# sony/aki

Measured on NVIDIA B200. Metric: mma_attn_fwd_bwd_tflops, higher is better.
Workload: dtype bf16

## Files before the change

### aki_b200/csrc/attn_bwd_sm100.cu

```cuda
#include <math.h>
#include <stdio.h>
#include <stdlib.h>
#include <mutex>
#include "attn_aux.cuh"
#include "sm100_ptx.cuh"

namespace aki {

namespace bwd {
constexpr int BN = 128, BM = 128;
constexpr int ATOM_BYTES = 128 * 64;
constexpr int TILE_BYTES = 3 * ATOM_BYTES;
constexpr int AUG_BYTES = 128 * 16;
constexpr int DQ_ATOM_BYTES = 128 * 128;
constexpr int Q_STAGES = 2, DO_STAGES = 2;
constexpr int THREADS = 512;
constexpr int MAX_TILES = 512;
constexpr int SMEM_K = 0;
constexpr int SMEM_V = SMEM_K + TILE_BYTES;
constexpr int SMEM_Q = SMEM_V + TILE_BYTES;
constexpr int SMEM_DO = SMEM_Q + Q_STAGES * TILE_BYTES;
constexpr int SMEM_DS = SMEM_DO + DO_STAGES * TILE_BYTES;
constexpr int SMEM_DQ = SMEM_DS + 4 * ATOM_BYTES;
constexpr int SMEM_QAUG = SMEM_DQ + 2 * DQ_ATOM_BYTES;
constexpr int SMEM_ONES = SMEM_QAUG + Q_STAGES * AUG_BYTES;
constexpr int SMEM_ONES_D = SMEM_ONES + 128;
constexpr int SMEM_ZERO = SMEM_ONES_D + 128;
constexpr int SLOTS = 2;
constexpr int SMEM_QLIST = SMEM_ZERO + 128;
constexpr int SMEM_TOTAL = SMEM_QLIST + SLOTS * MAX_TILES * 2;
#ifndef AKI_BWD_SLICES_PER_GROUP
#define AKI_BWD_SLICES_PER_GROUP 8
#endif
constexpr int SMEM_ALLOC = SMEM_TOTAL + 1024;
static_assert(SMEM_ALLOC + 256 <= 232448, "shared memory budget");
constexpr uint32_t TM_S = 0, TM_DP = 128, TM_DV = 256, TM_DK = 352, TM_P = 448;
constexpr int REGS_CTRL = 64, REGS_COMPUTE = 168, REGS_DRAIN = 112;
}

struct BwdKernelParams {
  TensorView d_k, d_v;
  const float* rope_cos;
  const float* rope_sin;
  int64_t rope_stride_b;
  MaskMeta mm;
  int B, H, T, n_t, n_words;
  int group, n_items, use_clc;
  float scale_log2, scale;
  unsigned long long* trace;
  int trace_cta;
};

#ifdef AKI_FWD_TRACE
#define TRB(slot, j, k) do { if (tracing && (j) < 64) P.trace[((slot) * 64 + (j)) * 8 + (k)] = clock64(); } while (0)
#else
#define TRB(slot, j, k) do { } while (0)
#endif

__device__ __forceinline__ void f32x2_mul(float& lo, float& hi, float a_lo, float a_hi, float b_lo, float b_hi) {
  uint64_t r;
  asm("mul.rn.f32x2 %0, %1, %2;" : "=l"(r) : "l"(f32x2_pack(a_lo, a_hi)), "l"(f32x2_pack(b_lo, b_hi)));
  asm("mov.b64 {%0, %1}, %2;" : "=f"(lo), "=f"(hi) : "l"(r));
}

__global__ void __launch_bounds__(bwd::THREADS, 1)
attn_bwd_sm100_kernel(const __grid_constant__ CUtensorMap map_q, const __grid_constant__ CUtensorMap map_k,
                      const __grid_constant__ CUtensorMap map_v, const __grid_constant__ CUtensorMap map_do,
                      const __grid_constant__ CUtensorMap map_dq, const __grid_constant__ CUtensorMap map_qaug,
                      const BwdKernelParams P) {
  using namespace bwd;
  extern __shared__ uint8_t smem_raw[];
  const uint32_t smem_base = (smem_u32(smem_raw) + 1023u) & ~1023u;
  uint8_t* const smem_gen = smem_raw + (smem_base - smem_u32(smem_raw));
  constexpr int KV_FULL = 0, KV_EMPTY = 1, Q_FULL = 2, Q_EMPTY = Q_FULL + Q_STAGES, DO_FULL = Q_EMPTY + Q_STAGES,
                DO_EMPTY = DO_FULL + DO_STAGES, S_FULL = DO_EMPTY + DO_STAGES, P_READY = S_FULL + 1,
                DP_FULL = P_READY + 1, DS_READY = DP_FULL + 1, DQ_FULL = DS_READY + 1, DQ_DRAINED = DQ_FULL + 1,
                ALL_DONE = DQ_DRAINED + 1, ACC_FREE = ALL_DONE + 1,
                ITEM_FULL = ACC_FREE + 1, ITEM_EMPTY = ITEM_FULL + SLOTS, CLC_BAR = ITEM_EMPTY + SLOTS, N_BARS = CLC_BAR + 1;
  __shared__ __align__(8) uint64_t bars[N_BARS];
  __shared__ __align__(16) int4 item_ring[SLOTS][2];
  __shared__ __align__(16) uint4 clc_resp;
  __shared__ uint32_t tmem_base_s;
  const uint32_t bar0 = smem_u32(bars);
  auto BAR = [&](int i) { return bar0 + 8u * i; };

  const int tid = threadIdx.x, warp = tid >> 5, lane = tid & 31;
  uint16_t* const qlist_all = reinterpret_cast<uint16_t*>(smem_gen + SMEM_QLIST);

  if (tid == 0) {
    mbar_init(BAR(KV_FULL), 1); mbar_init(BAR(KV_EMPTY), 2);
    for (int i = 0; i < Q_STAGES; ++i) { mbar_init(BAR(Q_FULL + i), 1); mbar_init(BAR(Q_EMPTY + i), 2); }
    for (int i = 0; i < DO_STAGES; ++i) { mbar_init(BAR(DO_FULL + i), 1); mbar_init(BAR(DO_EMPTY + i), 2); }
    mbar_init(BAR(S_FULL), 1); mbar_init(BAR(P_READY), 256); mbar_init(BAR(DP_FULL), 1);
    mbar_init(BAR(DS_READY), 256); mbar_init(BAR(DQ_FULL), 1); mbar_init(BAR(DQ_DRAINED), 128);
    mbar_init(BAR(ALL_DONE), 2); mbar_init(BAR(ACC_FREE), 256);
    for (int i = 0; i < SLOTS; ++i) { mbar_init(BAR(ITEM_FULL + i), 1); mbar_init(BAR(ITEM_EMPTY + i), 15); }
    mbar_init(BAR(CLC_BAR), 1);
    fence_barrier_init();
  }
  if (warp == 2) {
    tmem_alloc<512>(smem_u32(&tmem_base_s));
    if (lane < 8) *reinterpret_cast<uint4*>(smem_gen + SMEM_ONES + lane * 16) = make_uint4(0x3f803f80u, 0x00003f80u, 0u, 0u);
    else if (lane < 16) *reinterpret_cast<uint4*>(smem_gen + SMEM_ONES_D + (lane - 8) * 16) = make_uint4(0u, 0u, 0x3f803f80u, 0x00003f80u);
    else if (lane < 24) *reinterpret_cast<uint4*>(smem_gen + SMEM_ZERO + (lane - 16) * 16) = make_uint4(0u, 0u, 0u, 0u);
    fence_proxy_async_smem();
  }
  if (warp == 0 && elect_one()) {
    tma_prefetch_desc(&map_q); tma_prefetch_desc(&map_k); tma_prefetch_desc(&map_v); tma_prefetch_desc(&map_do);
    tma_prefetch_desc(&map_dq); tma_prefetch_desc(&map_qaug);
  }
  tc_fence_before();
  __syncthreads();
  tc_fence_after();
  const uint32_t tmem = tmem_base_s;

  auto item_wait = [&](uint32_t n, int4& v0, int4& v1) {
    const int slot = n % SLOTS;
    mbar_wait(BAR(ITEM_FULL + slot), (n / SLOTS) & 1);
    v0 = item_ring[slot][0]; v1 = item_ring[slot][1];
  };

  if (warp == 0) {
    setmaxnreg_dec<REGS_CTRL>();
    if (elect_one()) {
      uint32_t n_it = 0, n_work = 0, qc = 0;
      for (;;) {
        int4 v0, v1;
        item_wait(n_it, v0, v1);
        if (!v0.x) break;
        const int b = v0.y, h = v0.z, j0 = v0.w * BN, n_q = v1.x;
        const uint16_t* qlist = qlist_all + (n_it % SLOTS) * MAX_TILES;
        auto load_tile = [&](int it) {
          const int i0 = (int)qlist[it];
          const uint32_t c = qc + it, sq = c % Q_STAGES, sd = c % DO_STAGES;
          mbar_wait(BAR(Q_EMPTY + sq), ((c / Q_STAGES) & 1) ^ 1);
#ifdef KO_TMA
          if (c >= Q_STAGES) { mbar_arrive(BAR(Q_FULL + sq)); mbar_wait(BAR(DO_EMPTY + sd), ((c / DO_STAGES) & 1) ^ 1); mbar_arrive(BAR(DO_FULL + sd)); return; }
#endif
          mbar_arrive_expect_tx(BAR(Q_FULL + sq), TILE_BYTES + AUG_BYTES);
          for (int a = 0; a < 3; ++a)
            tma_load_4d(smem_base + SMEM_Q + sq * TILE_BYTES + a * ATOM_BYTES, &map_q, BAR(Q_FULL + sq), a * 32, i0, h, b);
          tma_load_4d(smem_base + SMEM_QAUG + sq * AUG_BYTES, &map_qaug, BAR(Q_FULL + sq), 0, i0, h, b);
          mbar_wait(BAR(DO_EMPTY + sd), ((c / DO_STAGES) & 1) ^ 1);
          mbar_arrive_expect_tx(BAR(DO_FULL + sd), TILE_BYTES);
          for (int a = 0; a < 3; ++a)
            tma_load_4d(smem_base + SMEM_DO + sd * TILE_BYTES + a * ATOM_BYTES, &map_do, BAR(DO_FULL + sd), a * 32, i0, h, b);
        };
        if (n_q > 0) {
          const int pre = min(n_q, Q_STAGES);
          for (int it = 0; it < pre; ++it) load_tile(it);
          if (n_work > 0) mbar_wait(BAR(KV_EMPTY), (n_work - 1) & 1);
          mbar_arrive_expect_tx(BAR(KV_FULL), 2 * TILE_BYTES);
          for (int a = 0; a < 3; ++a) {
            tma_load_4d(smem_base + SMEM_K + a * ATOM_BYTES, &map_k, BAR(KV_FULL), a * 32, j0, h, b);
            tma_load_4d(smem_base + SMEM_V + a * ATOM_BYTES, &map_v, BAR(KV_FULL), a * 32, j0, h, b);
          }
          for (int it = pre; it < n_q; ++it) load_tile(it);
          qc += n_q;
          ++n_work;
        }
        mbar_arrive(BAR(ITEM_EMPTY + n_it % SLOTS));
        ++n_it;
      }
    }
  } else if (warp == 1 || warp == 2) {
    setmaxnreg_dec<REGS_CTRL>();
    if (elect_one()) {
      constexpr uint32_t IDESC_SS_KK = umma_idesc_bf16(128, 128, 0, 0);
      constexpr uint32_t IDESC_N96_BMN = umma_idesc_bf16(128, 96, 0, 1);
      constexpr uint32_t IDESC_N96_AMN_BMN = umma_idesc_bf16(128, 96, 1, 1);
      const uint32_t sK = smem_base + SMEM_K, sV = smem_base + SMEM_V, sDS = smem_base + SMEM_DS;
      const uint64_t DESC_KMAJ = umma_smem_desc(0, 16, 512, UMMA_SW64);
      const uint64_t DESC_MNMAJ = umma_smem_desc(0, ATOM_BYTES, 512, UMMA_SW64);
      const uint64_t DESC_ONES = umma_smem_desc(smem_base + SMEM_ONES, SMEM_ZERO - SMEM_ONES, 0, UMMA_SW_NONE);
      const uint64_t DESC_ONES_D = umma_smem_desc(smem_base + SMEM_ONES_D, SMEM_ZERO - SMEM_ONES_D, 0, UMMA_SW_NONE);
      const uint64_t DESC_AUG = umma_smem_desc(0, 0, 128, UMMA_SW_NONE);
      auto kmajor = [&](uint32_t base, int k) {
        return DESC_KMAJ | (uint64_t)(((base + (k >> 1) * ATOM_BYTES + (k & 1) * 32) >> 4) & 0x3FFFu);
      };
      auto mnmajor = [&](uint32_t base, int k) {
        return DESC_MNMAJ | (uint64_t)(((base + k * 1024) >> 4) & 0x3FFFu);
      };
      uint32_t n_it = 0, n_work = 0, gs = 0;
      if (warp == 1) {
        for (;;) {
          int4 v0, v1;
          item_wait(n_it, v0, v1);
          if (!v0.x) break;
          const int n_q = v1.x;
#ifdef AKI_FWD_TRACE
          const bool tracing = P.trace && (int)blockIdx.x == P.trace_cta && n_it == 0;
#endif
          if (n_q > 0) {
          auto issue_s = [&](int it) {
            const uint32_t c = gs + it;
            const uint32_t sQ = smem_base + SMEM_Q + (c % Q_STAGES) * TILE_BYTES;
            const uint32_t sA = smem_base + SMEM_QAUG + (c % Q_STAGES) * AUG_BYTES;
#ifndef KO_S
#pragma unroll
            for (int k = 0; k < 6; ++k) umma_ss(tmem + TM_S, kmajor(sK, k), kmajor(sQ, k), IDESC_SS_KK, k > 0);
            umma_ss(tmem + TM_S, DESC_ONES, DESC_AUG | (uint64_t)((sA >> 4) & 0x3FFFu), IDESC_SS_KK, 1);
#endif
            umma_commit(BAR(S_FULL));
            umma_commit(BAR(Q_EMPTY + c % Q_STAGES));
          };
          mbar_wait(BAR(KV_FULL), n_work & 1);
          mbar_wait(BAR(Q_FULL + gs % Q_STAGES), (gs / Q_STAGES) & 1);
          tc_fence_after();
          issue_s(0);
          for (int it = 0; it < n_q; ++it) {
            const uint32_t c = gs + it;
            const uint32_t sDO = smem_base + SMEM_DO + (c % DO_STAGES) * TILE_BYTES;
            TRB(2, it, 0);
            mbar_wait(BAR(DO_FULL + c % DO_STAGES), (c / DO_STAGES) & 1);
            mbar_wait(BAR(P_READY), c & 1);
            if (it == 0 && n_work > 0) mbar_wait(BAR(ACC_FREE), (n_work - 1) & 1);
            tc_fence_after();
            TRB(2, it, 1);
#ifndef KO_DV
#pragma unroll
            for (int k = 0; k < 8; ++k)
              umma_ts(tmem + TM_DV, tmem + TM_P + 8 * k, mnmajor(sDO, k), IDESC_N96_BMN, (it > 0 || k > 0));
#endif
            umma_commit(BAR(DO_EMPTY + c % DO_STAGES));
            TRB(2, it, 2);
            if (it + 1 < n_q) {
              mbar_wait(BAR(Q_FULL + (c + 1) % Q_STAGES), ((c + 1) / Q_STAGES) & 1);
              tc_fence_after();
              TRB(2, it, 3);
              issue_s(it + 1);
              TRB(2, it, 4);
            }
          }
          umma_commit(BAR(ALL_DONE));
          umma_commit(BAR(KV_EMPTY));
            gs += n_q; ++n_work;
          }
          mbar_arrive(BAR(ITEM_EMPTY + n_it % SLOTS));
          ++n_it;
        }
      } else {
        for (;;) {
          int4 v0, v1;
          item_wait(n_it, v0, v1);
          if (!v0.x) break;
          const int n_q = v1.x;
#ifdef AKI_FWD_TRACE
          const bool tracing = P.trace && (int)blockIdx.x == P.trace_cta && n_it == 0;
#endif
          if (n_q > 0) {
          auto issue_dp = [&](int it) {
            const uint32_t c = gs + it;
            const uint32_t sDO = smem_base + SMEM_DO + (c % DO_STAGES) * TILE_BYTES;
            const uint32_t sA = smem_base + SMEM_QAUG + (c % Q_STAGES) * AUG_BYTES;
#ifndef KO_DP
#pragma unroll
            for (int k = 0; k < 6; ++k) umma_ss(tmem + TM_DP, kmajor(sV, k), kmajor(sDO, k), IDESC_SS_KK, k > 0);
            umma_ss(tmem + TM_DP, DESC_ONES_D, DESC_AUG | (uint64_t)((sA >> 4) & 0x3FFFu), IDESC_SS_KK, 1);
#endif
            umma_commit(BAR(DP_FULL));
            umma_commit(BAR(DO_EMPTY + c % DO_STAGES));
          };
          mbar_wait(BAR(KV_FULL), n_work & 1);
          mbar_wait(BAR(DO_FULL + gs % DO_STAGES), (gs / DO_STAGES) & 1);
          mbar_wait(BAR(Q_FULL + gs % Q_STAGES), (gs / Q_STAGES) & 1);
          if (gs > 0) mbar_wait(BAR(DQ_DRAINED), (gs - 1) & 1);
          tc_fence_after();
          issue_dp(0);
          for (int it = 0; it < n_q; ++it) {
            const uint32_t c = gs + it;
            const uint32_t sQ = smem_base + SMEM_Q + (c % Q_STAGES) * TILE_BYTES;
            TRB(3, it, 0);
            mbar_wait(BAR(DS_READY), c & 1);
            tc_fence_after();
            TRB(3, it, 1);
#ifndef KO_DQ
#pragma unroll
            for (int k = 0; k < 8; ++k)
              umma_ss(tmem + TM_DP, mnmajor(sDS, k), mnmajor(sK, k), IDESC_N96_AMN_BMN, k > 0);
#endif
            umma_commit(BAR(DQ_FULL));
            if (it == 0 && n_work > 0) { mbar_wait(BAR(ACC_FREE), (n_work - 1) & 1); tc_fence_after(); }
#ifndef KO_DK
#pragma unroll
            for (int k = 0; k < 8; ++k)
              umma_ss(tmem + TM_DK, kmajor(sDS, k), mnmajor(sQ, k), IDESC_N96_BMN, (it > 0 || k > 0));
#endif
            umma_commit(BAR(Q_EMPTY + c % Q_STAGES));
            TRB(3, it, 2);
            if (it + 1 < n_q) {
              mbar_wait(BAR(DO_FULL + (c + 1) % DO_STAGES), ((c + 1) / DO_STAGES) & 1);
              mbar_wait(BAR(Q_FULL + (c + 1) % Q_STAGES), ((c + 1) / Q_STAGES) & 1);
              TRB(3, it, 3);
              mbar_wait(BAR(DQ_DRAINED), c & 1);
              tc_fence_after();
              TRB(3, it, 4);
              issue_dp(it + 1);
              TRB(3, it, 5);
            }
          }
          umma_commit(BAR(ALL_DONE));
          umma_commit(BAR(KV_EMPTY));
            gs += n_q; ++n_work;
          }
          mbar_arrive(BAR(ITEM_EMPTY + n_it % SLOTS));
          ++n_it;
        }
      }
    }
  } else if (warp == 3) {
    setmaxnreg_dec<REGS_CTRL>();
    uint32_t n_pub = 0, n_clc = 0;
    long long id = blockIdx.x;
    for (;;) {
      const int per_group = P.n_t * P.group;
      const int g = (int)(id / per_group), rem = (int)(id % per_group);
      const int kt = rem / P.group, bh = g * P.group + rem % P.group;
      if (bh < P.B * P.H) {
        const int b = bh / P.H, h = bh % P.H;
        const int len = meta_len(P.mm, b, P.T);
        const int j0 = kt * BN;
        const int slot = n_pub % SLOTS;
        mbar_wait(BAR(ITEM_EMPTY + slot), ((n_pub / SLOTS) & 1) ^ 1);
        uint16_t* const qlist = qlist_all + slot * MAX_TILES;
        const int n_live = (len + BM - 1) / BM;
        int n = 0;
        if (j0 < len) {
          if (P.mm.kv_tile_q_mask) {
            const uint32_t* mrow = P.mm.kv_tile_q_mask + ((size_t)b * P.n_t + kt) * P.n_words;
            for (int w0 = 0; w0 < P.n_words; w0 += 32) {
              const int w = w0 + lane;
              uint32_t word = (w < P.n_words) ? mrow[w] : 0u;
              if (w * 32 >= n_live) word = 0u;
              else if (w * 32 + 32 > n_live) word &= (1u << (n_live - w * 32)) - 1u;
              const int cnt = __popc(word);
              int incl = cnt;
#pragma unroll
              for (int o = 1; o < 32; o <<= 1) {
                const int t = __shfl_up_sync(0xffffffffu, incl, o);
                if (lane >= o) incl += t;
              }
              int pos = n + incl - cnt;
              while (word) {
                const int bit = __ffs(word) - 1;
                word &= word - 1;
                qlist[pos++] = (uint16_t)((w * 32 + bit) * BM);
              }
              n += __shfl_sync(0xffffffffu, incl, 31);
            }
            __syncwarp();
            int n_pre = 0;
            for (int e = lane; e < n; e += 32) n_pre += ((int)qlist[e] < j0) ? 1 : 0;
#pragma unroll
            for (int o = 16; o > 0; o >>= 1) n_pre += __shfl_xor_sync(0xffffffffu, n_pre, o);
            if (n_pre >= 2 && P.mm.row_lo) {
              auto relevant = [&](int i) {
                if (i >= len) return false;
                const int lo = __ldg(P.mm.row_lo + (size_t)b * P.mm.meta_pitch + i);
                const int hi = __ldg(P.mm.row_hi + (size_t)b * P.mm.meta_pitch + i);
                return hi > lo && lo < j0 + BN && hi > j0;
              };
              int out = 0, e = 0;
              while (e < n_pre) {
                const int a = (int)qlist[e];
                int i0 = a, step = 1;
                if (e + 1 < n_pre && (int)qlist[e + 1] == a + BM) {
                  int first = 1 << 30, last = -1;
#pragma unroll
                  for (int k = 0; k < 4; ++k) {
                    const int row = 32 * k + lane;
                    if (relevant(a + row)) first = min(first, row);
                    if (relevant(a + BM + row)) last = max(last, row);
                  }
#pragma unroll
                  for (int o = 16; o > 0; o >>= 1) {
                    first = min(first, __shfl_xor_sync(0xffffffffu, first, o));
                    last = max(last, __shfl_xor_sync(0xffffffffu, last, o));
                  }
                  if (first > 0 && first < BM && last < first) { i0 = a + first; step = 2; }
                }
                __syncwarp();
                if (lane == 0) qlist[out] = (uint16_t)i0;
                ++out;
                e += step;
              }
              const int shift = n_pre - out;
              if (shift > 0) {
                for (int base = n_pre; base < n; base += 32) {
                  const int idx = base + lane;
                  const uint16_t v = (idx < n) ? qlist[idx] : (uint16_t)0;
                  __syncwarp();
                  if (idx < n) qlist[idx - shift] = v;
                  __syncwarp();
                }
                n -= shift;
              }
            }
          } else {
            for (int qt = kt + lane; qt < n_live; qt += 32) qlist[qt - kt] = (uint16_t)(qt * BM);
            n = max(0, n_live - kt);
          }
        }
        bool ok = true;
        if (lane < 4) {
          const int jw = j0 + 32 * lane;
          ok = (jw + 32 <= len);
          if (ok && P.mm.vbits) ok = (P.mm.vbits[(size_t)b * P.mm.bits_pitch + (jw >> 5)] == 0xffffffffu);
        }
        ok = __all_sync(0xffffffffu, ok);
        __syncwarp();
        if (lane == 0) {
          item_ring[slot][0] = make_int4(1, b, h, kt);
          item_ring[slot][1] = make_int4(n, ok ? 1 : 0, len, 0);
          mbar_arrive(BAR(ITEM_FULL + slot));
        }
        ++n_pub;
      }
      int more = 0;
      long long next = 0;
      if (lane == 0) {
        if (!P.use_clc) {
          next = id + gridDim.x;
          more = next < P.n_items;
        } else {
          mbar_arrive_expect_tx(BAR(CLC_BAR), 16);
          clc_try_cancel(smem_u32(&clc_resp), BAR(CLC_BAR));
          mbar_wait(BAR(CLC_BAR), n_clc & 1);
          uint32_t x;
          more = clc_query(smem_u32(&clc_resp), x) ? 1 : 0;
          next = x;
          fence_proxy_async_smem();
        }
      }
      ++n_clc;
      more = __shfl_sync(0xffffffffu, more, 0);
      next = __shfl_sync(0xffffffffu, next, 0);
      if (!more) break;
      id = next;
    }
    {
      const int slot = n_pub % SLOTS;
      mbar_wait(BAR(ITEM_EMPTY + slot), ((n_pub / SLOTS) & 1) ^ 1);
      if (lane == 0) {
        item_ring[slot][0] = make_int4(0, 0, 0, 0);
        item_ring[slot][1] = make_int4(0, 0, 0, 0);
        mbar_arrive(BAR(ITEM_FULL + slot));
      }
    }
  } else if (warp < 12) {
    setmaxnreg_inc<REGS_COMPUTE>();
    const int ct = tid - 128;
    const int r = ct & 127;
    const int hq = ct >> 7;
    const uint32_t lane_base = (uint32_t)((warp & 3) * 32) << 16;
    uint32_t n_it = 0, n_work = 0, gs = 0;
    for (;;) {
      int4 v0, v1;
      item_wait(n_it, v0, v1);
      if (!v0.x) break;
      const int b = v0.y, h = v0.z, j0 = v0.w * BN, n_q = v1.x, len = v1.z;
      const bool keys_all_valid = v1.y != 0;
      const uint16_t* qlist = qlist_all + (n_it % SLOTS) * MAX_TILES;
      const int j = j0 + r;

      bool k_valid = (j < len), k_mutual = (j < len);
      if (j < len && P.mm.vbits) k_valid = (P.mm.vbits[(size_t)b * P.mm.bits_pitch + (j >> 5)] >> (j & 31)) & 1u;
      if (j < len && P.mm.mbits) k_mutual = (P.mm.mbits[(size_t)b * P.mm.bits_pitch + (j >> 5)] >> (j & 31)) & 1u;

      float p[64];
#ifdef AKI_FWD_TRACE
      const bool tracing = P.trace && (int)blockIdx.x == P.trace_cta && (tid & 127) == 0 && n_it == 0;
      const int slot = hq;
#endif

      auto phase_a = [&](int it) {
        const uint32_t c = gs + it;
        const int i0 = (int)qlist[it];
        const bool full = (i0 >= j0 + BN) && keys_all_valid;
        TRB(slot, it, 0);
        mbar_wait(BAR(S_FULL), c & 1);
        tc_fence_after();
        TRB(slot, it, 1);
        uint32_t sraw[64];
        tmem_ld_x32(tmem + TM_S + lane_base + 64 * hq, sraw);
        tmem_ld_x32(tmem + TM_S + lane_base + 64 * hq + 32, sraw + 32);
        tmem_wait_ld();
#pragma unroll
        for (int c2 = 0; c2 < 64; c2 += 2) {
          float x0, x1;
          f32x2_mul(x0, x1, __uint_as_float(sraw[c2]), __uint_as_float(sraw[c2 + 1]), P.scale_log2, P.scale_log2);
#ifdef KO_EXP
          p[c2] = x0; p[c2 + 1] = x1;
#else
          p[c2] = ex2_approx(x0);
          p[c2 + 1] = ex2_approx(x1);
#endif
        }
        if (!full) {
          const int cmin = k_valid ? (j - i0 - 64 * hq) : (1 << 30);
          if (P.mm.row_lo && k_mutual) {
            const int32_t* lo_p = P.mm.row_lo + (size_t)b * P.mm.meta_pitch + i0 + 64 * hq;
            const int32_t* hi_p = P.mm.row_hi + (size_t)b * P.mm.meta_pitch + i0 + 64 * hq;
            const int n_live = len - (i0 + 64 * hq);
#pragma unroll
            for (int cc = 0; cc < 64; ++cc) {
              int lo = 0, wd = 0;
              if (cc < n_live) { lo = __ldg(lo_p + cc); wd = max(__ldg(hi_p + cc) - lo, 0); }
              const bool ok = (cc >= cmin) || ((unsigned)(j - lo) < (unsigned)wd);
              p[cc] = ok ? p[cc] : 0.f;
            }
          } else {
#pragma unroll
            for (int cc = 0; cc < 64; ++cc) p[cc] = (cc >= cmin) ? p[cc] : 0.f;
          }
        }
        uint32_t pk[32];
#pragma unroll
        for (int x = 0; x < 32; ++x) pk[x] = pack_bf16x2(p[2 * x], p[2 * x + 1]);
        TRB(slot, it, 2);
        tmem_st_x32(tmem + TM_P + lane_base + 32 * hq, pk);
        tmem_wait_st();
        tc_fence_before();
        mbar_arrive(BAR(P_READY));
        TRB(slot, it, 3);
      };

      auto phase_b = [&](int it) {
        const uint32_t c = gs + it;
        TRB(slot, it, 4);
        mbar_wait(BAR(DP_FULL), c & 1);
        tc_fence_after();
        TRB(slot, it, 5);
        uint32_t draw[64];
        tmem_ld_x32(tmem + TM_DP + lane_base + 64 * hq, draw);
        tmem_ld_x32(tmem + TM_DP + lane_base + 64 * hq + 32, draw + 32);
        tmem_wait_ld();
        const uint32_t ds_base = smem_base + SMEM_DS;
        uint32_t dsw[32];
#pragma unroll
        for (int c8 = 0; c8 < 8; ++c8) {
#pragma unroll
          for (int e = 0; e < 4; ++e) {
            const int cc = 8 * c8 + 2 * e;
            float d0, d1;
            f32x2_mul(d0, d1, p[cc], p[cc + 1], __uint_as_float(draw[cc]), __uint_as_float(draw[cc + 1]));
            dsw[4 * c8 + e] = pack_bf16x2(d0, d1);
          }
          const int col = 64 * hq + 8 * c8;
          const uint32_t addr = ds_base + (col >> 5) * ATOM_BYTES + sw64_offset(r, (col & 31) >> 3);
#ifndef KO_DS
          asm volatile("st.shared.v4.u32 [%0], {%1,%2,%3,%4};" ::"r"(addr), "r"(dsw[4 * c8]), "r"(dsw[4 * c8 + 1]),
                       "r"(dsw[4 * c8 + 2]), "r"(dsw[4 * c8 + 3]));
#endif
        }
#if !defined(KO_DS) && !defined(KO_FENCE)
        fence_proxy_async_smem();
#endif
        tc_fence_before();
        mbar_arrive(BAR(DS_READY));
        TRB(slot, it, 6);
      };

      for (int step = 0; step <= n_q && n_q > 0; ++step) {
        if (step > 0) phase_b(step - 1);
        if (step < n_q) phase_a(step);
      }

      {
        const bool store_row = (j < P.T);
        const int js = store_row ? j : 0;
        __nv_bfloat16* dvrow = P.d_v.row(b, js, h) + 48 * hq;
        __nv_bfloat16* dkrow = P.d_k.row(b, js, h);
        if (n_q > 0) {
          float cs[24], sn[24];
          if (P.rope_cos) {
            const float4* c4 = reinterpret_cast<const float4*>(P.rope_cos + (size_t)b * P.rope_stride_b + (size_t)js * 48 + 24 * hq);
            const float4* s4 = reinterpret_cast<const float4*>(P.rope_sin + (size_t)b * P.rope_stride_b + (size_t)js * 48 + 24 * hq);
#pragma unroll
            for (int x = 0; x < 6; ++x) {
              *reinterpret_cast<float4*>(cs + 4 * x) = __ldg(c4 + x);
              *reinterpret_cast<float4*>(sn + 4 * x) = __ldg(s4 + x);
            }
          }
          mbar_wait(BAR(ALL_DONE), n_work & 1);
          tc_fence_after();
          uint32_t acc[48];
          tmem_ld_x32(tmem + TM_DV + lane_base + 48 * hq, acc);
          tmem_ld_x16(tmem + TM_DV + lane_base + 48 * hq + 32, acc + 32);
          uint32_t lo[24], hi[24];
          tmem_ld_x16(tmem + TM_DK + lane_base + 24 * hq, lo);
          tmem_ld_x8(tmem + TM_DK + lane_base + 24 * hq + 16, *reinterpret_cast<uint32_t(*)[8]>(lo + 16));
          tmem_ld_x16(tmem + TM_DK + lane_base + 48 + 24 * hq, hi);
          tmem_ld_x8(tmem + TM_DK + lane_base + 48 + 24 * hq + 16, *reinterpret_cast<uint32_t(*)[8]>(hi + 16));
          tmem_wait_ld();
          tc_fence_before();
          mbar_arrive(BAR(ACC_FREE));
#pragma unroll
          for (int x = 0; x < 6; ++x) {
            uint4 u;
            u.x = pack_bf16x2(__uint_as_float(acc[8 * x]), __uint_as_float(acc[8 * x + 1]));
            u.y = pack_bf16x2(__uint_as_float(acc[8 * x + 2]), __uint_as_float(acc[8 * x + 3]));
            u.z = pack_bf16x2(__uint_as_float(acc[8 * x + 4]), __uint_as_float(acc[8 * x + 5]));
            u.w = pack_bf16x2(__uint_as_float(acc[8 * x + 6]), __uint_as_float(acc[8 * x + 7]));
            if (store_row) *reinterpret_cast<uint4*>(dvrow + 8 * x) = u;
          }
          float flo[24], fhi[24];
#pragma unroll
          for (int x = 0; x < 24; ++x) {
            float a = __uint_as_float(lo[x]) * P.scale, e = __uint_as_float(hi[x]) * P.scale;
            if (P.rope_cos) {
              const float a2 = a * cs[x] + e * sn[x], e2 = e * cs[x] - a * sn[x];
              a = a2; e = e2;
            }
            flo[x] = a; fhi[x] = e;
          }
#pragma unroll
          for (int x = 0; x < 3; ++x) {
            uint4 u, w;
            u.x = pack_bf16x2(flo[8 * x], flo[8 * x + 1]); u.y = pack_bf16x2(flo[8 * x + 2], flo[8 * x + 3]);
            u.z = pack_bf16x2(flo[8 * x + 4], flo[8 * x + 5]); u.w = pack_bf16x2(flo[8 * x + 6], flo[8 * x + 7]);
            w.x = pack_bf16x2(fhi[8 * x], fhi[8 * x + 1]); w.y = pack_bf16x2(fhi[8 * x + 2], fhi[8 * x + 3]);
            w.z = pack_bf16x2(fhi[8 * x + 4], fhi[8 * x + 5]); w.w = pack_bf16x2(fhi[8 * x + 6], fhi[8 * x + 7]);
            if (store_row) {
              *reinterpret_cast<uint4*>(dkrow + 24 * hq + 8 * x) = u;
              *reinterpret_cast<uint4*>(dkrow + 48 + 24 * hq + 8 * x) = w;
            }
          }
        } else if (store_row) {
          const uint4 z = make_uint4(0, 0, 0, 0);
#pragma unroll
          for (int x = 0; x < 6; ++x) *reinterpret_cast<uint4*>(dvrow + 8 * x) = z;
#pragma unroll
          for (int x = 0; x < 3; ++x) {
            *reinterpret_cast<uint4*>(dkrow + 24 * hq + 8 * x) = z;
            *reinterpret_cast<uint4*>(dkrow + 48 + 24 * hq + 8 * x) = z;
          }
        }
      }
      if (n_q > 0) { gs += n_q; ++n_work; }
      __syncwarp();
      if (lane == 0) mbar_arrive(BAR(ITEM_EMPTY + n_it % SLOTS));
      ++n_it;
    }
  } else {
    setmaxnreg_dec<REGS_DRAIN>();
    const int r = tid - 384;
    const uint32_t lane_base = (uint32_t)((warp & 3) * 32) << 16;
    uint32_t n_it = 0, gs = 0;
    for (;;) {
      int4 v0, v1;
      item_wait(n_it, v0, v1);
      if (!v0.x) break;
      const int b = v0.y, h = v0.z, n_q = v1.x;
      const uint16_t* qlist = qlist_all + (n_it % SLOTS) * MAX_TILES;
#ifdef AKI_FWD_TRACE
      const bool tracing = P.trace && (int)blockIdx.x == P.trace_cta && r == 0 && n_it == 0;
#endif
      for (int it = 0; it < n_q; ++it) {
        const uint32_t c = gs + it;
        const int i0 = (int)qlist[it];
        TRB(4, it, 0);
        mbar_wait(BAR(DQ_FULL), c & 1);
        tc_fence_after();
        TRB(4, it, 1);
#ifdef KO_DRAIN
        mbar_arrive(BAR(DQ_DRAINED));
        continue;
#endif
        uint32_t dq[96];
        tmem_ld_x32(tmem + TM_DP + lane_base, dq);
        tmem_ld_x32(tmem + TM_DP + lane_base + 32, dq + 32);
        tmem_ld_x32(tmem + TM_DP + lane_base + 64, dq + 64);
        tmem_wait_ld();
        tc_fence_before();
        mbar_arrive(BAR(DQ_DRAINED));
        TRB(4, it, 2);
#pragma unroll
        for (int a = 0; a < 3; ++a) {
          const int buf = (c * 3 + a) & 1;
          const uint32_t abase = smem_base + SMEM_DQ + buf * DQ_ATOM_BYTES;
          if (r == 0) tma_store_wait_read<1>();
          named_bar_sync(2, 128);
#pragma unroll
          for (int x = 0; x < 8; ++x) {
            const uint32_t addr = abase + r * 128 + ((x ^ (r & 7)) << 4);
            asm volatile("st.shared.v4.u32 [%0], {%1,%2,%3,%4};" ::"r"(addr), "r"(dq[32 * a + 4 * x]),
                         "r"(dq[32 * a + 4 * x + 1]), "r"(dq[32 * a + 4 * x + 2]), "r"(dq[32 * a + 4 * x + 3]) : "memory");
          }
          fence_proxy_async_smem();
          named_bar_sync(3, 128);
#ifndef KO_RED
          if (r == 0) {
            tma_reduce_add_4d(&map_dq, abase, 32 * a, i0, h, b);
            tma_store_commit();
          }
#endif
        }
      }
      gs += n_q;
      __syncwarp();
      if (lane == 0) mbar_arrive(BAR(ITEM_EMPTY + n_it % SLOTS));
      ++n_it;
    }
    if (r == 0) tma_store_wait_read<0>();
  }
  tc_fence_before();
  __syncthreads();
  if (warp == 2) tmem_dealloc<512>(tmem);
}

struct BwdDeviceState {
  std::once_flag once;
  int sm_count = 0;
  cudaError_t err = cudaSuccess;
};
static BwdDeviceState g_bwd_dev[64];

static int bwd_device_setup(int* sm_count) {
  int dev = 0;
  if (cudaGetDevice(&dev) != cudaSuccess || dev < 0 || dev >= 64) { set_last_cuda_error("cudaGetDevice failed"); return AKI_ERR_CUDA; }
  BwdDeviceState& s = g_bwd_dev[dev];
  std::call_once(s.once, [&]() {
    s.err = cudaFuncSetAttribute(attn_bwd_sm100_kernel, cudaFuncAttributeMaxDynamicSharedMemorySize, bwd::SMEM_ALLOC);
    if (s.err == cudaSuccess) s.err = cudaDeviceGetAttribute(&s.sm_count, cudaDevAttrMultiProcessorCount, dev);
  });
  if (s.err != cudaSuccess) { set_last_cuda_error(cudaGetErrorString(s.err)); return AKI_ERR_CUDA; }
  *sm_count = s.sm_count;
  return AKI_OK;
}

}

using namespace aki;

extern "C" int aki_mma_attn_bwd(const AkiMmaAttnBwdParams* p, aki_stream_t stream) {
  AKI_REQUIRE(p, AKI_ERR_NULL);
  const AkiMmaAttnParams& f = p->fwd;
  AKI_REQUIRE(f.q_offset == 0, AKI_ERR_UNSUPPORTED);
  int rc = check_attn_params(f);
  if (rc) return rc;
  if ((rc = check_tensor(p->d_o)) || (rc = check_tensor(p->d_q)) || (rc = check_tensor(p->d_k)) ||
      (rc = check_tensor(p->d_v)))
    return rc;
  AKI_REQUIRE(f.lse && p->workspace, AKI_ERR_NULL);
  AKI_REQUIRE(p->deterministic == 0, AKI_ERR_UNSUPPORTED);
  AKI_REQUIRE(p->workspace_bytes >= aki_mma_attn_bwd_workspace_bytes(f.B, f.H, f.T, f.D), AKI_ERR_BAD_SHAPE);
  AKI_REQUIRE((reinterpret_cast<uintptr_t>(p->workspace) & 255u) == 0, AKI_ERR_MISALIGNED);
  cudaStream_t st = static_cast<cudaStream_t>(stream);
  BwdWorkspace w = carve_bwd_workspace(p->workspace, f.B, f.H, f.T, f.D);
  if ((rc = launch_bwd_preprocess(*p, w, st))) return rc;
  if (cudaMemsetAsync(w.dq_accum, 0, (size_t)f.B * f.H * f.T * f.D * sizeof(float), st) != cudaSuccess) {
    set_last_cuda_error(cudaGetErrorString(cudaGetLastError()));
    return AKI_ERR_CUDA;
  }
  AkiMmaTensor4 qrot{w.q_rot, (int64_t)f.H * f.T * f.D, (int64_t)f.D, (int64_t)f.T * f.D};
  CUtensorMap mq, mk, mv, mdo, mdq, mqa;
  if ((rc = make_tile_map(&mq, qrot, f.B, f.H, f.T, bwd::BM))) return rc;
  if ((rc = make_tile_map(&mk, f.k, f.B, f.H, f.T, bwd::BN))) return rc;
  if ((rc = make_tile_map(&mv, f.v, f.B, f.H, f.T, bwd::BN))) return rc;
  if ((rc = make_tile_map(&mdo, p->d_o, f.B, f.H, f.T, bwd::BM))) return rc;
  if ((rc = make_dq_accum_map(&mdq, w.dq_accum, f.B, f.H, f.T))) return rc;
  if ((rc = make_row_stats_map(&mqa, w.row_stats, f.B, f.H, w.t_pad))) return rc;
  BwdKernelParams kp;
  kp.d_k = view_of(p->d_k); kp.d_v = view_of(p->d_v);
  kp.rope_cos = f.rope_cos; kp.rope_sin = f.rope_sin; kp.rope_stride_b = f.rope_stride_b;
  kp.mm = mask_meta_from(f);
  kp.B = f.B; kp.H = f.H; kp.T = f.T;
  kp.n_t = (f.T + bwd::BN - 1) / bwd::BN;
  kp.n_words = (kp.n_t + 31) / 32;
  AKI_REQUIRE(kp.n_t <= bwd::MAX_TILES, AKI_ERR_UNSUPPORTED);
  kp.scale = f.scale;
  kp.scale_log2 = f.scale * 1.4426950408889634f;
  kp.trace = nullptr; kp.trace_cta = -1;
#ifdef AKI_FWD_TRACE
  const char* trace_env = getenv("AKI_MMA_BWD_TRACE");
  const size_t trace_bytes = 5 * 64 * 8 * sizeof(unsigned long long);
  if (trace_env) {
    kp.trace_cta = atoi(trace_env);
    cudaMalloc(&kp.trace, trace_bytes);
    cudaMemset(kp.trace, 0, trace_bytes);
  }
#endif
  const long long slices = (long long)f.B * f.H;
  kp.group = (int)(slices < AKI_BWD_SLICES_PER_GROUP ? slices : AKI_BWD_SLICES_PER_GROUP);
  const long long n_groups = (slices + kp.group - 1) / kp.group;
  const long long n_items = n_groups * kp.n_t * kp.group;
  AKI_REQUIRE(n_items > 0 && n_items < (1ll << 31), AKI_ERR_BAD_SHAPE);
  kp.n_items = (int)n_items;
  int sm_count = 0;
  if ((rc = bwd_device_setup(&sm_count))) return rc;
  static const bool use_static = []() { const char* e = getenv("AKI_MMA_BWD_SCHED"); return e && e[0] == 's'; }();
  kp.use_clc = use_static ? 0 : 1;
  const long long grid = kp.use_clc ? n_items : (n_items < sm_count ? n_items : sm_count);
  timing_hook_begin(st);
  attn_bwd_sm100_kernel<<<(unsigned)grid, bwd::THREADS, bwd::SMEM_ALLOC, st>>>(mq, mk, mv, mdo, mdq, mqa, kp);
  timing_hook_end(st);
#ifdef AKI_FWD_TRACE
  if (trace_env) {
    cudaDeviceSynchronize();
    static unsigned long long host[5 * 64 * 8];
    cudaMemcpy(host, kp.trace, trace_bytes, cudaMemcpyDeviceToHost);
    cudaFree(kp.trace);
    unsigned long long t0 = ~0ull;
    for (size_t i = 0; i < 5 * 64 * 8; ++i) if (host[i] && host[i] < t0) t0 = host[i];
    const char* names[5] = {"cmp_h0", "cmp_h1", "mma_A", "mma_B", "drain"};
    for (int slot = 0; slot < 5; ++slot)
      for (int j = 0; j < 64; ++j) {
        bool any = false;
        for (int k = 0; k < 8; ++k) any = any || host[(slot * 64 + j) * 8 + k];
        if (!any) continue;
        fprintf(stderr, "TRACE %s it=%d:", names[slot], j);
        for (int k = 0; k < 7; ++k) fprintf(stderr, " %llu", host[(slot * 64 + j) * 8 + k] ? host[(slot * 64 + j) * 8 + k] - t0 : 0ull);
        fprintf(stderr, "\n");
      }
  }
#endif
  if ((rc = check_launch())) return rc;
  return launch_dq_finalize(*p, w, f.scale, st);
}
```

### aki_b200/csrc/sm100_ptx.cuh

```cuda
#pragma once
#include <cuda.h>
#include <cuda_bf16.h>
#include <cuda_runtime.h>
#include <stdint.h>

namespace aki {

__device__ __forceinline__ uint32_t smem_u32(const void* p) {
  return static_cast<uint32_t>(__cvta_generic_to_shared(p));
}
__device__ __forceinline__ bool elect_one() {
  uint32_t pred = 0;
  asm volatile(
      "{\n\t.reg .pred P;\n\telect.sync _|P, 0xffffffff;\n\tselp.b32 %0, 1, 0, P;\n\t}\n"
      : "=r"(pred));
  return pred != 0;
}

__device__ __forceinline__ void mbar_init(uint32_t bar, uint32_t count) {
  asm volatile("mbarrier.init.shared::cta.b64 [%0], %1;" ::"r"(bar), "r"(count));
}
__device__ __forceinline__ void fence_barrier_init() {
  asm volatile("fence.mbarrier_init.release.cluster;" ::: "memory");
}
__device__ __forceinline__ void mbar_arrive(uint32_t bar) {
  asm volatile("mbarrier.arrive.shared::cta.b64 _, [%0];" ::"r"(bar) : "memory");
}
__device__ __forceinline__ void mbar_arrive_expect_tx(uint32_t bar, uint32_t bytes) {
  asm volatile("mbarrier.arrive.expect_tx.shared::cta.b64 _, [%0], %1;" ::"r"(bar), "r"(bytes) : "memory");
}
__device__ __forceinline__ bool mbar_try_wait(uint32_t bar, uint32_t parity) {
  uint32_t ok;
  asm volatile(
      "{\n\t.reg .pred P;\n\t"
      "mbarrier.try_wait.parity.shared::cta.b64 P, [%1], %2;\n\t"
      "selp.b32 %0, 1, 0, P;\n\t}\n"
      : "=r"(ok)
      : "r"(bar), "r"(parity)
      : "memory");
  return ok != 0;
}
__device__ __forceinline__ bool mbar_test(uint32_t bar, uint32_t parity) {
  uint32_t ok;
  asm volatile(
      "{\n\t.reg .pred P;\n\t"
      "mbarrier.test_wait.parity.shared::cta.b64 P, [%1], %2;\n\t"
      "selp.b32 %0, 1, 0, P;\n\t}\n"
      : "=r"(ok)
      : "r"(bar), "r"(parity)
      : "memory");
  return ok != 0;
}
#ifndef AKI_MBAR_TRAP_NS
#define AKI_MBAR_TRAP_NS 4000000000ull
#endif
#ifndef AKI_MBAR_SUSPEND_NS
#define AKI_MBAR_SUSPEND_NS 0x989680u
#endif
__device__ __forceinline__ bool mbar_try_wait_hint(uint32_t bar, uint32_t parity) {
  uint32_t ok;
  asm volatile(
      "{\n\t.reg .pred P;\n\t"
      "mbarrier.try_wait.parity.shared::cta.b64 P, [%1], %2, %3;\n\t"
      "selp.b32 %0, 1, 0, P;\n\t}\n"
      : "=r"(ok)
      : "r"(bar), "r"(parity), "r"(AKI_MBAR_SUSPEND_NS)
      : "memory");
  return ok != 0;
}
__device__ __forceinline__ void mbar_wait(uint32_t bar, uint32_t parity) {
#ifdef AKI_MBAR_TRAP
  unsigned long long t0 = 0, now;
  while (!mbar_try_wait_hint(bar, parity)) {
    asm volatile("mov.u64 %0, %%globaltimer;" : "=l"(now));
    if (t0 == 0) t0 = now;
    else if (now - t0 > AKI_MBAR_TRAP_NS) __trap();
  }
#else
  while (!mbar_try_wait_hint(bar, parity)) { }
#endif
}

__device__ __forceinline__ void clc_try_cancel(uint32_t resp_smem, uint32_t bar) {
  asm volatile("clusterlaunchcontrol.try_cancel.async.shared::cta.mbarrier::complete_tx::bytes.b128 [%0], [%1];" ::"r"(
                   resp_smem),
               "r"(bar)
               : "memory");
}
__device__ __forceinline__ bool clc_query(uint32_t resp_smem, uint32_t& cta_x) {
  uint32_t valid = 0, x = 0;
  asm volatile(
      "{\n\t.reg .pred p1;\n\t.reg .b128 resp;\n\t"
      "ld.shared.b128 resp, [%2];\n\t"
      "clusterlaunchcontrol.query_cancel.is_canceled.pred.b128 p1, resp;\n\t"
      "selp.u32 %1, 1, 0, p1;\n\t"
      "@p1 clusterlaunchcontrol.query_cancel.get_first_ctaid::x.b32.b128 %0, resp;\n\t}\n"
      : "=r"(x), "=r"(valid)
      : "r"(resp_smem)
      : "memory");
  cta_x = x;
  return valid != 0;
}

__device__ __forceinline__ void fence_proxy_async_smem() {
  asm volatile("fence.proxy.async.shared::cta;" ::: "memory");
}
__device__ __forceinline__ void tc_fence_before() { asm volatile("tcgen05.fence::before_thread_sync;" ::: "memory"); }
__device__ __forceinline__ void tc_fence_after() { asm volatile("tcgen05.fence::after_thread_sync;" ::: "memory"); }
__device__ __forceinline__ void named_bar_sync(int id, int nthreads) {
  asm volatile("bar.sync %0, %1;" ::"r"(id), "r"(nthreads) : "memory");
}

__device__ __forceinline__ void tma_prefetch_desc(const CUtensorMap* m) {
  asm volatile("prefetch.tensormap [%0];" ::"l"(reinterpret_cast<uint64_t>(m)) : "memory");
}
__device__ __forceinline__ void tma_load_4d(uint32_t dst, const CUtensorMap* m, uint32_t bar, int c0, int c1, int c2,
                                            int c3) {
  asm volatile(
      "cp.async.bulk.tensor.4d.shared::cluster.global.mbarrier::complete_tx::bytes [%0], [%1, {%3, %4, %5, %6}], [%2];"
      ::"r"(dst), "l"(reinterpret_cast<uint64_t>(m)), "r"(bar), "r"(c0), "r"(c1), "r"(c2), "r"(c3)
      : "memory");
}
__device__ __forceinline__ void tma_store_4d(const CUtensorMap* m, uint32_t src, int c0, int c1, int c2, int c3) {
  asm volatile("cp.async.bulk.tensor.4d.global.shared::cta.bulk_group [%0, {%2, %3, %4, %5}], [%1];" ::"l"(
                   reinterpret_cast<uint64_t>(m)),
               "r"(src), "r"(c0), "r"(c1), "r"(c2), "r"(c3)
               : "memory");
}
__device__ __forceinline__ void tma_reduce_add_4d(const CUtensorMap* m, uint32_t src, int c0, int c1, int c2, int c3) {
  asm volatile("cp.reduce.async.bulk.tensor.4d.global.shared::cta.add.bulk_group [%0, {%2, %3, %4, %5}], [%1];" ::"l"(
                   reinterpret_cast<uint64_t>(m)),
               "r"(src), "r"(c0), "r"(c1), "r"(c2), "r"(c3)
               : "memory");
}
__device__ __forceinline__ void tma_store_commit() { asm volatile("cp.async.bulk.commit_group;" ::: "memory"); }
template <int N>
__device__ __forceinline__ void tma_store_wait_read() {
  asm volatile("cp.async.bulk.wait_group.read %0;" ::"n"(N) : "memory");
}
template <int N>
__device__ __forceinline__ void tma_store_wait() {
  asm volatile("cp.async.bulk.wait_group %0;" ::"n"(N) : "memory");
}

template <int NCOLS>
__device__ __forceinline__ void tmem_alloc(uint32_t dst_smem) {
  asm volatile("tcgen05.alloc.cta_group::1.sync.aligned.shared::cta.b32 [%0], %1;" ::"r"(dst_smem), "n"(NCOLS)
               : "memory");
  asm volatile("tcgen05.relinquish_alloc_permit.cta_group::1.sync.aligned;" ::: "memory");
}
template <int NCOLS>
__device__ __forceinline__ void tmem_dealloc(uint32_t taddr) {
  asm volatile("tcgen05.dealloc.cta_group::1.sync.aligned.b32 %0, %1;" ::"r"(taddr), "n"(NCOLS) : "memory");
}
__device__ __forceinline__ void tmem_wait_ld() { asm volatile("tcgen05.wait::ld.sync.aligned;" ::: "memory"); }
__device__ __forceinline__ void tmem_wait_st() { asm volatile("tcgen05.wait::st.sync.aligned;" ::: "memory"); }

__device__ __forceinline__ void tmem_ld_x8(uint32_t taddr, uint32_t (&r)[8]) {
  asm volatile("tcgen05.ld.sync.aligned.32x32b.x8.b32 {%0,%1,%2,%3,%4,%5,%6,%7}, [%8];"
               : "=r"(r[0]), "=r"(r[1]), "=r"(r[2]), "=r"(r[3]), "=r"(r[4]), "=r"(r[5]), "=r"(r[6]), "=r"(r[7])
               : "r"(taddr));
}
__device__ __forceinline__ void tmem_ld_x16(uint32_t taddr, uint32_t* r) {
  asm volatile(
      "tcgen05.ld.sync.aligned.32x32b.x16.b32 {%0,%1,%2,%3,%4,%5,%6,%7,%8,%9,%10,%11,%12,%13,%14,%15}, [%16];"
      : "=r"(r[0]), "=r"(r[1]), "=r"(r[2]), "=r"(r[3]), "=r"(r[4]), "=r"(r[5]), "=r"(r[6]), "=r"(r[7]), "=r"(r[8]),
        "=r"(r[9]), "=r"(r[10]), "=r"(r[11]), "=r"(r[12]), "=r"(r[13]), "=r"(r[14]), "=r"(r[15])
      : "r"(taddr));
}
__device__ __forceinline__ void tmem_ld_x32(uint32_t taddr, uint32_t* r) {
  asm volatile(
      "tcgen05.ld.sync.aligned.32x32b.x32.b32 "
      "{%0,%1,%2,%3,%4,%5,%6,%7,%8,%9,%10,%11,%12,%13,%14,%15,%16,%17,%18,%19,%20,%21,%22,%23,%24,%25,%26,%27,%28,%29,"
      "%30,%31}, [%32];"
      : "=r"(r[0]), "=r"(r[1]), "=r"(r[2]), "=r"(r[3]), "=r"(r[4]), "=r"(r[5]), "=r"(r[6]), "=r"(r[7]), "=r"(r[8]),
        "=r"(r[9]), "=r"(r[10]), "=r"(r[11]), "=r"(r[12]), "=r"(r[13]), "=r"(r[14]), "=r"(r[15]), "=r"(r[16]),
        "=r"(r[17]), "=r"(r[18]), "=r"(r[19]), "=r"(r[20]), "=r"(r[21]), "=r"(r[22]), "=r"(r[23]), "=r"(r[24]),
        "=r"(r[25]), "=r"(r[26]), "=r"(r[27]), "=r"(r[28]), "=r"(r[29]), "=r"(r[30]), "=r"(r[31])
      : "r"(taddr));
}
__device__ __forceinline__ void tmem_st_x8(uint32_t taddr, const uint32_t* r) {
  asm volatile("tcgen05.st.sync.aligned.32x32b.x8.b32 [%0], {%1,%2,%3,%4,%5,%6,%7,%8};" ::"r"(taddr), "r"(r[0]),
               "r"(r[1]), "r"(r[2]), "r"(r[3]), "r"(r[4]), "r"(r[5]), "r"(r[6]), "r"(r[7])
               : "memory");
}
__device__ __forceinline__ void tmem_st_x16(uint32_t taddr, const uint32_t* r) {
  asm volatile(
      "tcgen05.st.sync.aligned.32x32b.x16.b32 [%0], {%1,%2,%3,%4,%5,%6,%7,%8,%9,%10,%11,%12,%13,%14,%15,%16};" ::"r"(
          taddr),
      "r"(r[0]), "r"(r[1]), "r"(r[2]), "r"(r[3]), "r"(r[4]), "r"(r[5]), "r"(r[6]), "r"(r[7]), "r"(r[8]), "r"(r[9]),
      "r"(r[10]), "r"(r[11]), "r"(r[12]), "r"(r[13]), "r"(r[14]), "r"(r[15])
      : "memory");
}
__device__ __forceinline__ void tmem_st_x32(uint32_t taddr, const uint32_t* r) {
  asm volatile(
      "tcgen05.st.sync.aligned.32x32b.x32.b32 [%0], "
      "{%1,%2,%3,%4,%5,%6,%7,%8,%9,%10,%11,%12,%13,%14,%15,%16,%17,%18,%19,%20,%21,%22,%23,%24,%25,%26,%27,%28,%29,%30,"
      "%31,%32};" ::"r"(taddr),
      "r"(r[0]), "r"(r[1]), "r"(r[2]), "r"(r[3]), "r"(r[4]), "r"(r[5]), "r"(r[6]), "r"(r[7]), "r"(r[8]), "r"(r[9]),
      "r"(r[10]), "r"(r[11]), "r"(r[12]), "r"(r[13]), "r"(r[14]), "r"(r[15]), "r"(r[16]), "r"(r[17]), "r"(r[18]),
      "r"(r[19]), "r"(r[20]), "r"(r[21]), "r"(r[22]), "r"(r[23]), "r"(r[24]), "r"(r[25]), "r"(r[26]), "r"(r[27]),
      "r"(r[28]), "r"(r[29]), "r"(r[30]), "r"(r[31])
      : "memory");
}

enum : uint32_t { UMMA_SW_NONE = 0, UMMA_SW128 = 2, UMMA_SW64 = 4, UMMA_SW32 = 6 };
__device__ __forceinline__ uint64_t umma_smem_desc(uint32_t saddr, uint32_t lbo_bytes, uint32_t sbo_bytes,
                                                   uint32_t layout) {
  uint32_t lo = ((saddr >> 4) & 0x3FFFu) | (((lbo_bytes >> 4) & 0x3FFFu) << 16);
  uint32_t hi = ((sbo_bytes >> 4) & 0x3FFFu) | (1u << 14) | (layout << 29);
  return (static_cast<uint64_t>(hi) << 32) | lo;
}
__host__ __device__ constexpr uint32_t umma_idesc_bf16(int M, int N, int a_mn_major, int b_mn_major) {
  return (1u << 4) | (1u << 7) | (1u << 10) | (static_cast<uint32_t>(a_mn_major) << 15) |
         (static_cast<uint32_t>(b_mn_major) << 16) | (static_cast<uint32_t>(N >> 3) << 17) |
         (static_cast<uint32_t>(M >> 4) << 24);
}
__device__ __forceinline__ void umma_ss(uint32_t d_tmem, uint64_t adesc, uint64_t bdesc, uint32_t idesc,
                                        uint32_t accumulate) {
  asm volatile(
      "{\n\t.reg .pred p;\n\tsetp.ne.b32 p, %4, 0;\n\t"
      "tcgen05.mma.cta_group::1.kind::f16 [%0], %1, %2, %3, p;\n\t}\n" ::"r"(d_tmem),
      "l"(adesc), "l"(bdesc), "r"(idesc), "r"(accumulate)
      : "memory");
}
__device__ __forceinline__ void umma_ts(uint32_t d_tmem, uint32_t a_tmem, uint64_t bdesc, uint32_t idesc,
                                        uint32_t accumulate) {
  asm volatile(
      "{\n\t.reg .pred p;\n\tsetp.ne.b32 p, %4, 0;\n\t"
      "tcgen05.mma.cta_group::1.kind::f16 [%0], [%1], %2, %3, p;\n\t}\n" ::"r"(d_tmem),
      "r"(a_tmem), "l"(bdesc), "r"(idesc), "r"(accumulate)
      : "memory");
}
__device__ __forceinline__ void umma_commit(uint32_t bar) {
  asm volatile("tcgen05.commit.cta_group::1.mbarrier::arrive::one.shared::cluster.b64 [%0];" ::"r"(bar) : "memory");
}

template <int N>
__device__ __forceinline__ void setmaxnreg_inc() { asm volatile("setmaxnreg.inc.sync.aligned.u32 %0;" ::"n"(N)); }
template <int N>
__device__ __forceinline__ void setmaxnreg_dec() { asm volatile("setmaxnreg.dec.sync.aligned.u32 %0;" ::"n"(N)); }

__device__ __forceinline__ float ex2_approx(float x) {
  float y;
  asm("ex2.approx.ftz.f32 %0, %1;" : "=f"(y) : "f"(x));
  return y;
}
__device__ __forceinline__ uint32_t pack_bf16x2(float lo, float hi) {
  uint32_t r;
  asm("cvt.rn.bf16x2.f32 %0, %1, %2;" : "=r"(r) : "f"(hi), "f"(lo));
  return r;
}

__host__ __device__ __forceinline__ uint32_t sw64_offset(uint32_t r, uint32_t c) {
  return r * 64u + ((c ^ ((r >> 1) & 3u)) << 4);
}

__device__ __forceinline__ uint64_t f32x2_pack(float lo, float hi) {
  uint64_t r;
  asm("mov.b64 %0, {%1, %2};" : "=l"(r) : "f"(lo), "f"(hi));
  return r;
}
__device__ __forceinline__ void f32x2_unpack(uint64_t v, float& lo, float& hi) {
  asm("mov.b64 {%0, %1}, %2;" : "=f"(lo), "=f"(hi) : "l"(v));
}
__device__ __forceinline__ uint64_t f32x2_fma(uint64_t a, uint64_t b, uint64_t c) {
  uint64_t r;
  asm("fma.rn.f32x2 %0, %1, %2, %3;" : "=l"(r) : "l"(a), "l"(b), "l"(c));
  return r;
}
__device__ __forceinline__ uint64_t f32x2_add(uint64_t a, uint64_t b) {
  uint64_t r;
  asm("add.rn.f32x2 %0, %1, %2;" : "=l"(r) : "l"(a), "l"(b));
  return r;
}
__device__ __forceinline__ float fmax3(float a, float b, float c) {
  float r;
  asm("max.f32 %0, %1, %2, %3;" : "=f"(r) : "f"(a), "f"(b), "f"(c));
  return r;
}

}
```

Baseline: 822.6.

## Pair adjacent KV tiles in 2-CTA clusters and multicast shared Q/dO loads

Launches the backward kernel as 2-CTA clusters where each CTA owns one of two adjacent KV tiles. Both CTAs walk the union of Q tiles, and rank 0 multicasts Q while rank 1 multicasts dO into both CTAs' shared memory. Tiles that only one CTA needs are consumed as pass-through, releasing their buffers through multicast commits. The CLC scheduler is shared across the cluster. This is meant to halve global/L2 traffic for Q and dO, at the cost of cross-CTA lockstep coupling and wasted loads for tiles only one CTA uses.

```diff
diff --git a/aki_b200/csrc/attn_bwd_sm100.cu b/aki_b200/csrc/attn_bwd_sm100.cu
--- a/aki_b200/csrc/attn_bwd_sm100.cu
+++ b/aki_b200/csrc/attn_bwd_sm100.cu
@@ -28,7 +28,10 @@
 constexpr int SMEM_ZERO = SMEM_ONES_D + 128;
 constexpr int SLOTS = 2;
 constexpr int SMEM_QLIST = SMEM_ZERO + 128;
-constexpr int SMEM_TOTAL = SMEM_QLIST + SLOTS * MAX_TILES * 2;
+constexpr int SMEM_OLIST = SMEM_QLIST + SLOTS * MAX_TILES * 2;
+constexpr int SMEM_OFLAG = SMEM_OLIST + SLOTS * MAX_TILES * 2;
+constexpr int SMEM_TOTAL = SMEM_OFLAG + SLOTS * MAX_TILES;
+constexpr uint16_t PAIR_MASK = 0x3;
 #ifndef AKI_BWD_SLICES_PER_GROUP
 #define AKI_BWD_SLICES_PER_GROUP 8
 #endif
@@ -76,7 +79,8 @@
                 DO_EMPTY = DO_FULL + DO_STAGES, S_FULL = DO_EMPTY + DO_STAGES, P_READY = S_FULL + 1,
                 DP_FULL = P_READY + 1, DS_READY = DP_FULL + 1, DQ_FULL = DS_READY + 1, DQ_DRAINED = DQ_FULL + 1,
                 ALL_DONE = DQ_DRAINED + 1, ACC_FREE = ALL_DONE + 1,
-                ITEM_FULL = ACC_FREE + 1, ITEM_EMPTY = ITEM_FULL + SLOTS, CLC_BAR = ITEM_EMPTY + SLOTS, N_BARS = CLC_BAR + 1;
+                ITEM_FULL = ACC_FREE + 1, ITEM_EMPTY = ITEM_FULL + SLOTS, CLC_BAR = ITEM_EMPTY + SLOTS,
+                CLC_EMPTY = CLC_BAR + 1, N_BARS = CLC_EMPTY + 1;
   __shared__ __align__(8) uint64_t bars[N_BARS];
   __shared__ __align__(16) int4 item_ring[SLOTS][2];
   __shared__ __align__(16) uint4 clc_resp;
@@ -85,17 +89,20 @@
   auto BAR = [&](int i) { return bar0 + 8u * i; };
 
   const int tid = threadIdx.x, warp = tid >> 5, lane = tid & 31;
+  const uint32_t rank = cluster_ctarank();
   uint16_t* const qlist_all = reinterpret_cast<uint16_t*>(smem_gen + SMEM_QLIST);
+  uint16_t* const olist_all = reinterpret_cast<uint16_t*>(smem_gen + SMEM_OLIST);
+  uint8_t* const oflag_all = smem_gen + SMEM_OFLAG;
 
   if (tid == 0) {
     mbar_init(BAR(KV_FULL), 1); mbar_init(BAR(KV_EMPTY), 2);
-    for (int i = 0; i < Q_STAGES; ++i) { mbar_init(BAR(Q_FULL + i), 1); mbar_init(BAR(Q_EMPTY + i), 2); }
-    for (int i = 0; i < DO_STAGES; ++i) { mbar_init(BAR(DO_FULL + i), 1); mbar_init(BAR(DO_EMPTY + i), 2); }
+    for (int i = 0; i < Q_STAGES; ++i) { mbar_init(BAR(Q_FULL + i), 1); mbar_init(BAR(Q_EMPTY + i), 4); }
+    for (int i = 0; i < DO_STAGES; ++i) { mbar_init(BAR(DO_FULL + i), 1); mbar_init(BAR(DO_EMPTY + i), 4); }
     mbar_init(BAR(S_FULL), 1); mbar_init(BAR(P_READY), 256); mbar_init(BAR(DP_FULL), 1);
     mbar_init(BAR(DS_READY), 256); mbar_init(BAR(DQ_FULL), 1); mbar_init(BAR(DQ_DRAINED), 128);
     mbar_init(BAR(ALL_DONE), 2); mbar_init(BAR(ACC_FREE), 256);
     for (int i = 0; i < SLOTS; ++i) { mbar_init(BAR(ITEM_FULL + i), 1); mbar_init(BAR(ITEM_EMPTY + i), 15); }
-    mbar_init(BAR(CLC_BAR), 1);
+    mbar_init(BAR(CLC_BAR), 1); mbar_init(BAR(CLC_EMPTY), 2);
     fence_barrier_init();
   }
   if (warp == 2) {
@@ -110,7 +117,7 @@
     tma_prefetch_desc(&map_dq); tma_prefetch_desc(&map_qaug);
   }
   tc_fence_before();
-  __syncthreads();
+  cluster_sync();
   tc_fence_after();
   const uint32_t tmem = tmem_base_s;
 
@@ -128,7 +135,7 @@
         int4 v0, v1;
         item_wait(n_it, v0, v1);
         if (!v0.x) break;
-        const int b = v0.y, h = v0.z, j0 = v0.w * BN, n_q = v1.x;
+        const int b = v0.y, h = v0.z, j0 = v0.w * BN, n_q = v1.x, n_own = v1.w;
         const uint16_t* qlist = qlist_all + (n_it % SLOTS) * MAX_TILES;
         auto load_tile = [&](int it) {
           const int i0 = (int)qlist[it];
@@ -138,30 +145,40 @@
           if (c >= Q_STAGES) { mbar_arrive(BAR(Q_FULL + sq)); mbar_wait(BAR(DO_EMPTY + sd), ((c / DO_STAGES) & 1) ^ 1); mbar_arrive(BAR(DO_FULL + sd)); return; }
 #endif
           mbar_arrive_expect_tx(BAR(Q_FULL + sq), TILE_BYTES + AUG_BYTES);
-          for (int a = 0; a < 3; ++a)
-            tma_load_4d(smem_base + SMEM_Q + sq * TILE_BYTES + a * ATOM_BYTES, &map_q, BAR(Q_FULL + sq), a * 32, i0, h, b);
-          tma_load_4d(smem_base + SMEM_QAUG + sq * AUG_BYTES, &map_qaug, BAR(Q_FULL + sq), 0, i0, h, b);
+          if (rank == 0) {
+            for (int a = 0; a < 3; ++a)
+              tma_load_4d_multicast(smem_base + SMEM_Q + sq * TILE_BYTES + a * ATOM_BYTES, &map_q, BAR(Q_FULL + sq),
+                                    PAIR_MASK, a * 32, i0, h, b);
+            tma_load_4d_multicast(smem_base + SMEM_QAUG + sq * AUG_BYTES, &map_qaug, BAR(Q_FULL + sq), PAIR_MASK, 0, i0, h, b);
+          }
           mbar_wait(BAR(DO_EMPTY + sd), ((c / DO_STAGES) & 1) ^ 1);
           mbar_arrive_expect_tx(BAR(DO_FULL + sd), TILE_BYTES);
-          for (int a = 0; a < 3; ++a)
-            tma_load_4d(smem_base + SMEM_DO + sd * TILE_BYTES + a * ATOM_BYTES, &map_do, BAR(DO_FULL + sd), a * 32, i0, h, b);
+          if (rank == 1) {
+            for (int a = 0; a < 3; ++a)
+              tma_load_4d_multicast(smem_base + SMEM_DO + sd * TILE_BYTES + a * ATOM_BYTES, &map_do, BAR(DO_FULL + sd),
+                                    PAIR_MASK, a * 32, i0, h, b);
+          }
         };
         if (n_q > 0) {
           const int pre = min(n_q, Q_STAGES);
           for (int it = 0; it < pre; ++it) load_tile(it);
-          if (n_work > 0) mbar_wait(BAR(KV_EMPTY), (n_work - 1) & 1);
-          mbar_arrive_expect_tx(BAR(KV_FULL), 2 * TILE_BYTES);
-          for (int a = 0; a < 3; ++a) {
-            tma_load_4d(smem_base + SMEM_K + a * ATOM_BYTES, &map_k, BAR(KV_FULL), a * 32, j0, h, b);
-            tma_load_4d(smem_base + SMEM_V + a * ATOM_BYTES, &map_v, BAR(KV_FULL), a * 32, j0, h, b);
+          if (n_own > 0) {
+            if (n_work > 0) mbar_wait(BAR(KV_EMPTY), (n_work - 1) & 1);
+            mbar_arrive_expect_tx(BAR(KV_FULL), 2 * TILE_BYTES);
+            for (int a = 0; a < 3; ++a) {
+              tma_load_4d(smem_base + SMEM_K + a * ATOM_BYTES, &map_k, BAR(KV_FULL), a * 32, j0, h, b);
+              tma_load_4d(smem_base + SMEM_V + a * ATOM_BYTES, &map_v, BAR(KV_FULL), a * 32, j0, h, b);
+            }
+            ++n_work;
           }
           for (int it = pre; it < n_q; ++it) load_tile(it);
           qc += n_q;
-          ++n_work;
         }
         mbar_arrive(BAR(ITEM_EMPTY + n_it % SLOTS));
         ++n_it;
       }
+      for (uint32_t c = qc; c < qc + Q_STAGES; ++c) mbar_wait(BAR(Q_EMPTY + c % Q_STAGES), ((c / Q_STAGES) & 1) ^ 1);
+      for (uint32_t c = qc; c < qc + DO_STAGES; ++c) mbar_wait(BAR(DO_EMPTY + c % DO_STAGES), ((c / DO_STAGES) & 1) ^ 1);
     }
   } else if (warp == 1 || warp == 2) {
     setmaxnreg_dec<REGS_CTRL>();
@@ -181,19 +198,18 @@
       auto mnmajor = [&](uint32_t base, int k) {
         return DESC_MNMAJ | (uint64_t)(((base + k * 1024) >> 4) & 0x3FFFu);
       };
-      uint32_t n_it = 0, n_work = 0, gs = 0;
+      uint32_t n_it = 0, n_work = 0, qc = 0, gs = 0;
       if (warp == 1) {
         for (;;) {
           int4 v0, v1;
           item_wait(n_it, v0, v1);
           if (!v0.x) break;
-          const int n_q = v1.x;
+          const int n_q = v1.x, n_own = v1.w;
+          const uint8_t* oflag = oflag_all + (n_it % SLOTS) * MAX_TILES;
 #ifdef AKI_FWD_TRACE
           const bool tracing = P.trace && (int)blockIdx.x == P.trace_cta && n_it == 0;
 #endif
-          if (n_q > 0) {
-          auto issue_s = [&](int it) {
-            const uint32_t c = gs + it;
+          auto issue_s = [&](uint32_t c) {
             const uint32_t sQ = smem_base + SMEM_Q + (c % Q_STAGES) * TILE_BYTES;
             const uint32_t sA = smem_base + SMEM_QAUG + (c % Q_STAGES) * AUG_BYTES;
 #ifndef KO_S
@@ -202,18 +218,14 @@
             umma_ss(tmem + TM_S, DESC_ONES, DESC_AUG | (uint64_t)((sA >> 4) & 0x3FFFu), IDESC_SS_KK, 1);
 #endif
             umma_commit(BAR(S_FULL));
-            umma_commit(BAR(Q_EMPTY + c % Q_STAGES));
+            umma_commit_multicast(BAR(Q_EMPTY + c % Q_STAGES), PAIR_MASK);
           };
-          mbar_wait(BAR(KV_FULL), n_work & 1);
-          mbar_wait(BAR(Q_FULL + gs % Q_STAGES), (gs / Q_STAGES) & 1);
-          tc_fence_after();
-          issue_s(0);
-          for (int it = 0; it < n_q; ++it) {
-            const uint32_t c = gs + it;
+          auto issue_dv = [&](uint32_t c, int it) {
+            const uint32_t w = gs + it;
             const uint32_t sDO = smem_base + SMEM_DO + (c % DO_STAGES) * TILE_BYTES;
             TRB(2, it, 0);
             mbar_wait(BAR(DO_FULL + c % DO_STAGES), (c / DO_STAGES) & 1);
-            mbar_wait(BAR(P_READY), c & 1);
+            mbar_wait(BAR(P_READY), w & 1);
             if (it == 0 && n_work > 0) mbar_wait(BAR(ACC_FREE), (n_work - 1) & 1);
             tc_fence_after();
             TRB(2, it, 1);
@@ -222,20 +234,36 @@
             for (int k = 0; k < 8; ++k)
               umma_ts(tmem + TM_DV, tmem + TM_P + 8 * k, mnmajor(sDO, k), IDESC_N96_BMN, (it > 0 || k > 0));
 #endif
-            umma_commit(BAR(DO_EMPTY + c % DO_STAGES));
+            umma_commit_multicast(BAR(DO_EMPTY + c % DO_STAGES), PAIR_MASK);
             TRB(2, it, 2);
-            if (it + 1 < n_q) {
-              mbar_wait(BAR(Q_FULL + (c + 1) % Q_STAGES), ((c + 1) / Q_STAGES) & 1);
+          };
+          if (n_own > 0) mbar_wait(BAR(KV_FULL), n_work & 1);
+          int wi = 0;
+          bool prev_own = false;
+          for (int e = 0; e <= n_q; ++e) {
+            const uint32_t c = qc + e;
+            if (prev_own) issue_dv(c - 1, wi - 1);
+            if (e == n_q) break;
+            mbar_wait(BAR(Q_FULL + c % Q_STAGES), (c / Q_STAGES) & 1);
+            prev_own = oflag[e] != 0;
+            if (prev_own) {
               tc_fence_after();
-              TRB(2, it, 3);
-              issue_s(it + 1);
-              TRB(2, it, 4);
-            }
-          }
-          umma_commit(BAR(ALL_DONE));
-          umma_commit(BAR(KV_EMPTY));
-            gs += n_q; ++n_work;
-          }
+              if (wi > 0) TRB(2, wi - 1, 3);
+              issue_s(c);
+              if (wi > 0) TRB(2, wi - 1, 4);
+              ++wi;
+            } else {
+              mbar_wait(BAR(DO_FULL + c % DO_STAGES), (c / DO_STAGES) & 1);
+              umma_commit_multicast(BAR(Q_EMPTY + c % Q_STAGES), PAIR_MASK);
+              umma_commit_multicast(BAR(DO_EMPTY + c % DO_STAGES), PAIR_MASK);
+            }
+          }
+          if (n_own > 0) {
+            umma_commit(BAR(ALL_DONE));
+            umma_commit(BAR(KV_EMPTY));
+            ++n_work;
+          }
+          qc += n_q; gs += n_own;
           mbar_arrive(BAR(ITEM_EMPTY + n_it % SLOTS));
           ++n_it;
         }
@@ -244,13 +272,12 @@
           int4 v0, v1;
           item_wait(n_it, v0, v1);
           if (!v0.x) break;
-          const int n_q = v1.x;
+          const int n_q = v1.x, n_own = v1.w;
+          const uint8_t* oflag = oflag_all + (n_it % SLOTS) * MAX_TILES;
 #ifdef AKI_FWD_TRACE
           const bool tracing = P.trace && (int)blockIdx.x == P.trace_cta && n_it == 0;
 #endif
-          if (n_q > 0) {
-          auto issue_dp = [&](int it) {
-            const uint32_t c = gs + it;
+          auto issue_dp = [&](uint32_t c) {
             const uint32_t sDO = smem_base + SMEM_DO + (c % DO_STAGES) * TILE_BYTES;
             const uint32_t sA = smem_base + SMEM_QAUG + (c % Q_STAGES) * AUG_BYTES;
 #ifndef KO_DP
@@ -259,19 +286,13 @@
             umma_ss(tmem + TM_DP, DESC_ONES_D, DESC_AUG | (uint64_t)((sA >> 4) & 0x3FFFu), IDESC_SS_KK, 1);
 #endif
             umma_commit(BAR(DP_FULL));
-            umma_commit(BAR(DO_EMPTY + c % DO_STAGES));
+            umma_commit_multicast(BAR(DO_EMPTY + c % DO_STAGES), PAIR_MASK);
           };
-          mbar_wait(BAR(KV_FULL), n_work & 1);
-          mbar_wait(BAR(DO_FULL + gs % DO_STAGES), (gs / DO_STAGES) & 1);
-          mbar_wait(BAR(Q_FULL + gs % Q_STAGES), (gs / Q_STAGES) & 1);
-          if (gs > 0) mbar_wait(BAR(DQ_DRAINED), (gs - 1) & 1);
-          tc_fence_after();
-          issue_dp(0);
-          for (int it = 0; it < n_q; ++it) {
-            const uint32_t c = gs + it;
+          auto issue_dq_dk = [&](uint32_t c, int it) {
+            const uint32_t w = gs + it;
             const uint32_t sQ = smem_base + SMEM_Q + (c % Q_STAGES) * TILE_BYTES;
             TRB(3, it, 0);
-            mbar_wait(BAR(DS_READY), c & 1);
+            mbar_wait(BAR(DS_READY), w & 1);
             tc_fence_after();
             TRB(3, it, 1);
 #ifndef KO_DQ
@@ -286,23 +307,38 @@
             for (int k = 0; k < 8; ++k)
               umma_ss(tmem + TM_DK, kmajor(sDS, k), mnmajor(sQ, k), IDESC_N96_BMN, (it > 0 || k > 0));
 #endif
-            umma_commit(BAR(Q_EMPTY + c % Q_STAGES));
+            umma_commit_multicast(BAR(Q_EMPTY + c % Q_STAGES), PAIR_MASK);
             TRB(3, it, 2);
-            if (it + 1 < n_q) {
-              mbar_wait(BAR(DO_FULL + (c + 1) % DO_STAGES), ((c + 1) / DO_STAGES) & 1);
-              mbar_wait(BAR(Q_FULL + (c + 1) % Q_STAGES), ((c + 1) / Q_STAGES) & 1);
-              TRB(3, it, 3);
-              mbar_wait(BAR(DQ_DRAINED), c & 1);
+          };
+          if (n_own > 0) mbar_wait(BAR(KV_FULL), n_work & 1);
+          int wi = 0;
+          bool prev_own = false;
+          for (int e = 0; e <= n_q; ++e) {
+            const uint32_t c = qc + e;
+            if (prev_own) issue_dq_dk(c - 1, wi - 1);
+            if (e == n_q) break;
+            mbar_wait(BAR(DO_FULL + c % DO_STAGES), (c / DO_STAGES) & 1);
+            mbar_wait(BAR(Q_FULL + c % Q_STAGES), (c / Q_STAGES) & 1);
+            prev_own = oflag[e] != 0;
+            if (prev_own) {
+              if (wi > 0) TRB(3, wi - 1, 3);
+              if (gs + wi > 0) mbar_wait(BAR(DQ_DRAINED), (gs + wi - 1) & 1);
               tc_fence_after();
-              TRB(3, it, 4);
-              issue_dp(it + 1);
-              TRB(3, it, 5);
-            }
-          }
-          umma_commit(BAR(ALL_DONE));
-          umma_commit(BAR(KV_EMPTY));
-            gs += n_q; ++n_work;
-          }
+              if (wi > 0) TRB(3, wi - 1, 4);
+              issue_dp(c);
+              if (wi > 0) TRB(3, wi - 1, 5);
+              ++wi;
+            } else {
+              umma_commit_multicast(BAR(Q_EMPTY + c % Q_STAGES), PAIR_MASK);
+              umma_commit_multicast(BAR(DO_EMPTY + c % DO_STAGES), PAIR_MASK);
+            }
+          }
+          if (n_own > 0) {
+            umma_commit(BAR(ALL_DONE));
+            umma_commit(BAR(KV_EMPTY));
+            ++n_work;
+          }
+          qc += n_q; gs += n_own;
           mbar_arrive(BAR(ITEM_EMPTY + n_it % SLOTS));
           ++n_it;
         }
@@ -311,28 +347,37 @@
   } else if (warp == 3) {
     setmaxnreg_dec<REGS_CTRL>();
     uint32_t n_pub = 0, n_clc = 0;
-    long long id = blockIdx.x;
+    long long id = blockIdx.x >> 1;
     for (;;) {
-      const int per_group = P.n_t * P.group;
+      const int n_kp = (P.n_t + 1) >> 1;
+      const int per_group = n_kp * P.group;
       const int g = (int)(id / per_group), rem = (int)(id % per_group);
-      const int kt = rem / P.group, bh = g * P.group + rem % P.group;
+      const int kp = rem / P.group, bh = g * P.group + rem % P.group;
       if (bh < P.B * P.H) {
         const int b = bh / P.H, h = bh % P.H;
         const int len = meta_len(P.mm, b, P.T);
-        const int j0 = kt * BN;
+        const int kt0 = 2 * kp, kt = kt0 + (int)rank;
+        const int j0 = kt0 * BN, jo = kt * BN;
+        const bool own_live = kt < P.n_t && jo < len;
         const int slot = n_pub % SLOTS;
         mbar_wait(BAR(ITEM_EMPTY + slot), ((n_pub / SLOTS) & 1) ^ 1);
         uint16_t* const qlist = qlist_all + slot * MAX_TILES;
+        uint16_t* const olist = olist_all + slot * MAX_TILES;
+        uint8_t* const oflag = oflag_all + slot * MAX_TILES;
         const int n_live = (len + BM - 1) / BM;
-        int n = 0;
+        int n = 0, n_own = 0;
         if (j0 < len) {
           if (P.mm.kv_tile_q_mask) {
-            const uint32_t* mrow = P.mm.kv_tile_q_mask + ((size_t)b * P.n_t + kt) * P.n_words;
+            const uint32_t* mrow0 = P.mm.kv_tile_q_mask + ((size_t)b * P.n_t + kt0) * P.n_words;
+            const bool live1 = kt0 + 1 < P.n_t && j0 + BN < len;
             for (int w0 = 0; w0 < P.n_words; w0 += 32) {
               const int w = w0 + lane;
-              uint32_t word = (w < P.n_words) ? mrow[w] : 0u;
-              if (w * 32 >= n_live) word = 0u;
-              else if (w * 32 + 32 > n_live) word &= (1u << (n_live - w * 32)) - 1u;
+              uint32_t word0 = (w < P.n_words) ? mrow0[w] : 0u;
+              uint32_t word1 = (w < P.n_words && live1) ? mrow0[P.n_words + w] : 0u;
+              if (w * 32 >= n_live) { word0 = 0u; word1 = 0u; }
+              else if (w * 32 + 32 > n_live) { word0 &= (1u << (n_live - w * 32)) - 1u; word1 &= (1u << (n_live - w * 32)) - 1u; }
+              uint32_t word = word0 | word1;
+              const uint32_t mine = !own_live ? 0u : (rank ? word1 : word0);
               const int cnt = __popc(word);
               int incl = cnt;
 #pragma unroll
@@ -344,7 +389,8 @@
               while (word) {
                 const int bit = __ffs(word) - 1;
                 word &= word - 1;
-                qlist[pos++] = (uint16_t)((w * 32 + bit) * BM);
+                qlist[pos] = (uint16_t)((w * 32 + bit) * BM);
+                oflag[pos++] = (uint8_t)((mine >> bit) & 1u);
               }
               n += __shfl_sync(0xffffffffu, incl, 31);
             }
@@ -358,12 +404,13 @@
                 if (i >= len) return false;
                 const int lo = __ldg(P.mm.row_lo + (size_t)b * P.mm.meta_pitch + i);
                 const int hi = __ldg(P.mm.row_hi + (size_t)b * P.mm.meta_pitch + i);
-                return hi > lo && lo < j0 + BN && hi > j0;
+                return hi > lo && lo < j0 + 2 * BN && hi > j0;
               };
               int out = 0, e = 0;
               while (e < n_pre) {
                 const int a = (int)qlist[e];
                 int i0 = a, step = 1;
+                uint8_t flag = oflag[e];
                 if (e + 1 < n_pre && (int)qlist[e + 1] == a + BM) {
                   int first = 1 << 30, last = -1;
 #pragma unroll
@@ -377,10 +424,10 @@
                     first = min(first, __shfl_xor_sync(0xffffffffu, first, o));
                     last = max(last, __shfl_xor_sync(0xffffffffu, last, o));
                   }
-                  if (first > 0 && first < BM && last < first) { i0 = a + first; step = 2; }
+                  if (first > 0 && first < BM && last < first) { i0 = a + first; step = 2; flag |= oflag[e + 1]; }
                 }
                 __syncwarp();
-                if (lane == 0) qlist[out] = (uint16_t)i0;
+                if (lane == 0) { qlist[out] = (uint16_t)i0; oflag[out] = flag; }
                 ++out;
                 e += step;
               }
@@ -389,21 +436,36 @@
                 for (int base = n_pre; base < n; base += 32) {
                   const int idx = base + lane;
                   const uint16_t v = (idx < n) ? qlist[idx] : (uint16_t)0;
+                  const uint8_t f = (idx < n) ? oflag[idx] : (uint8_t)0;
                   __syncwarp();
-                  if (idx < n) qlist[idx - shift] = v;
+                  if (idx < n) { qlist[idx - shift] = v; oflag[idx - shift] = f; }
                   __syncwarp();
                 }
                 n -= shift;
               }
             }
+            __syncwarp();
+            for (int base = 0; base < n; base += 32) {
+              const int idx = base + lane;
+              const bool f = idx < n && oflag[idx] != 0;
+              const uint32_t bal = __ballot_sync(0xffffffffu, f);
+              if (f) olist[n_own + __popc(bal & ((1u << lane) - 1u))] = qlist[idx];
+              n_own += __popc(bal);
+            }
           } else {
-            for (int qt = kt + lane; qt < n_live; qt += 32) qlist[qt - kt] = (uint16_t)(qt * BM);
-            n = max(0, n_live - kt);
+            for (int qt = kt0 + lane; qt < n_live; qt += 32) {
+              const bool mine = own_live && qt >= kt;
+              qlist[qt - kt0] = (uint16_t)(qt * BM);
+              oflag[qt - kt0] = mine ? 1 : 0;
+              if (mine) olist[qt - kt] = (uint16_t)(qt * BM);
+            }
+            n = max(0, n_live - kt0);
+            n_own = own_live ? max(0, n_live - kt) : 0;
           }
         }
         bool ok = true;
         if (lane < 4) {
-          const int jw = j0 + 32 * lane;
+          const int jw = jo + 32 * lane;
           ok = (jw + 32 <= len);
           if (ok && P.mm.vbits) ok = (P.mm.vbits[(size_t)b * P.mm.bits_pitch + (jw >> 5)] == 0xffffffffu);
         }
@@ -411,7 +473,7 @@
         __syncwarp();
         if (lane == 0) {
           item_ring[slot][0] = make_int4(1, b, h, kt);
-          item_ring[slot][1] = make_int4(n, ok ? 1 : 0, len, 0);
+          item_ring[slot][1] = make_int4(n, ok ? 1 : 0, len, n_own);
           mbar_arrive(BAR(ITEM_FULL + slot));
         }
         ++n_pub;
@@ -420,16 +482,18 @@
       long long next = 0;
       if (lane == 0) {
         if (!P.use_clc) {
-          next = id + gridDim.x;
+          next = id + (gridDim.x >> 1);
           more = next < P.n_items;
         } else {
+          if (rank == 0 && n_clc > 0) mbar_wait(BAR(CLC_EMPTY), (n_clc - 1) & 1);
           mbar_arrive_expect_tx(BAR(CLC_BAR), 16);
-          clc_try_cancel(smem_u32(&clc_resp), BAR(CLC_BAR));
+          if (rank == 0) clc_try_cancel_multicast(smem_u32(&clc_resp), BAR(CLC_BAR));
           mbar_wait(BAR(CLC_BAR), n_clc & 1);
           uint32_t x;
           more = clc_query(smem_u32(&clc_resp), x) ? 1 : 0;
-          next = x;
+          next = x >> 1;
           fence_proxy_async_smem();
+          if (more) mbar_arrive_cluster(BAR(CLC_EMPTY), 0);
         }
       }
       ++n_clc;
@@ -458,9 +522,9 @@
       int4 v0, v1;
       item_wait(n_it, v0, v1);
       if (!v0.x) break;
-      const int b = v0.y, h = v0.z, j0 = v0.w * BN, n_q = v1.x, len = v1.z;
+      const int b = v0.y, h = v0.z, j0 = v0.w * BN, n_q = v1.w, len = v1.z;
       const bool keys_all_valid = v1.y != 0;
-      const uint16_t* qlist = qlist_all + (n_it % SLOTS) * MAX_TILES;
+      const uint16_t* qlist = olist_all + (n_it % SLOTS) * MAX_TILES;
       const int j = j0 + r;
 
       bool k_valid = (j < len), k_mutual = (j < len);
@@ -651,8 +715,8 @@
       int4 v0, v1;
       item_wait(n_it, v0, v1);
       if (!v0.x) break;
-      const int b = v0.y, h = v0.z, n_q = v1.x;
-      const uint16_t* qlist = qlist_all + (n_it % SLOTS) * MAX_TILES;
+      const int b = v0.y, h = v0.z, n_q = v1.w;
+      const uint16_t* qlist = olist_all + (n_it % SLOTS) * MAX_TILES;
 #ifdef AKI_FWD_TRACE
       const bool tracing = P.trace && (int)blockIdx.x == P.trace_cta && r == 0 && n_it == 0;
 #endif
@@ -705,27 +769,46 @@
     if (r == 0) tma_store_wait_read<0>();
   }
   tc_fence_before();
-  __syncthreads();
+  cluster_sync();
   if (warp == 2) tmem_dealloc<512>(tmem);
 }
 
+static void bwd_launch_config(cudaLaunchConfig_t* cfg, cudaLaunchAttribute* attr, unsigned grid, cudaStream_t st) {
+  *cfg = cudaLaunchConfig_t{};
+  cfg->gridDim = dim3(grid);
+  cfg->blockDim = dim3(bwd::THREADS);
+  cfg->dynamicSmemBytes = bwd::SMEM_ALLOC;
+  cfg->stream = st;
+  attr->id = cudaLaunchAttributeClusterDimension;
+  attr->val.clusterDim.x = 2; attr->val.clusterDim.y = 1; attr->val.clusterDim.z = 1;
+  cfg->attrs = attr;
+  cfg->numAttrs = 1;
+}
+
 struct BwdDeviceState {
   std::once_flag once;
-  int sm_count = 0;
+  int max_clusters = 0;
   cudaError_t err = cudaSuccess;
 };
 static BwdDeviceState g_bwd_dev[64];
 
-static int bwd_device_setup(int* sm_count) {
+static int bwd_device_setup(int* max_clusters) {
   int dev = 0;
   if (cudaGetDevice(&dev) != cudaSuccess || dev < 0 || dev >= 64) { set_last_cuda_error("cudaGetDevice failed"); return AKI_ERR_CUDA; }
   BwdDeviceState& s = g_bwd_dev[dev];
   std::call_once(s.once, [&]() {
     s.err = cudaFuncSetAttribute(attn_bwd_sm100_kernel, cudaFuncAttributeMaxDynamicSharedMemorySize, bwd::SMEM_ALLOC);
-    if (s.err == cudaSuccess) s.err = cudaDeviceGetAttribute(&s.sm_count, cudaDevAttrMultiProcessorCount, dev);
+    if (s.err != cudaSuccess) return;
+    cudaLaunchConfig_t cfg;
+    cudaLaunchAttribute attr;
+    bwd_launch_config(&cfg, &attr, 2, 0);
+    s.err = cudaOccupancyMaxActiveClusters(&s.max_clusters, attn_bwd_sm100_kernel, &cfg);
+    if (s.err == cudaSuccess && s.max_clusters < 1) s.err = cudaErrorInvalidConfiguration;
+    const char* v = getenv("AKI_MMA_BWD_VERBOSE");
+    if (v && v[0] == '1') fprintf(stderr, "attn_bwd_sm100_kernel: device %d fits %d clusters of 2 CTAs\n", dev, s.max_clusters);
   });
   if (s.err != cudaSuccess) { set_last_cuda_error(cudaGetErrorString(s.err)); return AKI_ERR_CUDA; }
-  *sm_count = s.sm_count;
+  *max_clusters = s.max_clusters;
   return AKI_OK;
 }
 
@@ -784,17 +867,21 @@
   const long long slices = (long long)f.B * f.H;
   kp.group = (int)(slices < AKI_BWD_SLICES_PER_GROUP ? slices : AKI_BWD_SLICES_PER_GROUP);
   const long long n_groups = (slices + kp.group - 1) / kp.group;
-  const long long n_items = n_groups * kp.n_t * kp.group;
-  AKI_REQUIRE(n_items > 0 && n_items < (1ll << 31), AKI_ERR_BAD_SHAPE);
+  const long long n_items = n_groups * ((kp.n_t + 1) / 2) * kp.group;
+  AKI_REQUIRE(n_items > 0 && n_items < (1ll << 30), AKI_ERR_BAD_SHAPE);
   kp.n_items = (int)n_items;
-  int sm_count = 0;
-  if ((rc = bwd_device_setup(&sm_count))) return rc;
+  int max_clusters = 0;
+  if ((rc = bwd_device_setup(&max_clusters))) return rc;
   static const bool use_static = []() { const char* e = getenv("AKI_MMA_BWD_SCHED"); return e && e[0] == 's'; }();
   kp.use_clc = use_static ? 0 : 1;
-  const long long grid = kp.use_clc ? n_items : (n_items < sm_count ? n_items : sm_count);
+  const long long clusters = kp.use_clc ? n_items : (n_items < max_clusters ? n_items : max_clusters);
+  cudaLaunchConfig_t cfg;
+  cudaLaunchAttribute attr;
+  bwd_launch_config(&cfg, &attr, (unsigned)(2 * clusters), st);
   timing_hook_begin(st);
-  attn_bwd_sm100_kernel<<<(unsigned)grid, bwd::THREADS, bwd::SMEM_ALLOC, st>>>(mq, mk, mv, mdo, mdq, mqa, kp);
+  const cudaError_t le = cudaLaunchKernelEx(&cfg, attn_bwd_sm100_kernel, mq, mk, mv, mdo, mdq, mqa, kp);
   timing_hook_end(st);
+  if (le != cudaSuccess) { set_last_cuda_error(cudaGetErrorString(le)); return AKI_ERR_CUDA; }
 #ifdef AKI_FWD_TRACE
   if (trace_env) {
     cudaDeviceSynchronize();
diff --git a/aki_b200/csrc/sm100_ptx.cuh b/aki_b200/csrc/sm100_ptx.cuh
--- a/aki_b200/csrc/sm100_ptx.cuh
+++ b/aki_b200/csrc/sm100_ptx.cuh
@@ -87,6 +87,13 @@
                "r"(bar)
                : "memory");
 }
+__device__ __forceinline__ void clc_try_cancel_multicast(uint32_t resp_smem, uint32_t bar) {
+  asm volatile(
+      "clusterlaunchcontrol.try_cancel.async.shared::cta.mbarrier::complete_tx::bytes.multicast::cluster::all.b128 "
+      "[%0], [%1];" ::"r"(resp_smem),
+      "r"(bar)
+      : "memory");
+}
 __device__ __forceinline__ bool clc_query(uint32_t resp_smem, uint32_t& cta_x) {
   uint32_t valid = 0, x = 0;
   asm volatile(
@@ -102,6 +109,22 @@
   return valid != 0;
 }
 
+__device__ __forceinline__ uint32_t cluster_ctarank() {
+  uint32_t r;
+  asm volatile("mov.u32 %0, %%cluster_ctarank;" : "=r"(r));
+  return r;
+}
+__device__ __forceinline__ void cluster_sync() {
+  asm volatile("barrier.cluster.arrive.release;\n\tbarrier.cluster.wait.acquire;" ::: "memory");
+}
+__device__ __forceinline__ void mbar_arrive_cluster(uint32_t bar, uint32_t cta) {
+  asm volatile(
+      "{\n\t.reg .b32 ra;\n\tmapa.shared::cluster.u32 ra, %0, %1;\n\t"
+      "mbarrier.arrive.release.cluster.shared::cluster.b64 _, [ra];\n\t}\n" ::"r"(bar),
+      "r"(cta)
+      : "memory");
+}
+
 __device__ __forceinline__ void fence_proxy_async_smem() {
   asm volatile("fence.proxy.async.shared::cta;" ::: "memory");
 }
@@ -119,6 +142,14 @@
   asm volatile(
       "cp.async.bulk.tensor.4d.shared::cluster.global.mbarrier::complete_tx::bytes [%0], [%1, {%3, %4, %5, %6}], [%2];"
       ::"r"(dst), "l"(reinterpret_cast<uint64_t>(m)), "r"(bar), "r"(c0), "r"(c1), "r"(c2), "r"(c3)
+      : "memory");
+}
+__device__ __forceinline__ void tma_load_4d_multicast(uint32_t dst, const CUtensorMap* m, uint32_t bar, uint16_t cta_mask,
+                                                      int c0, int c1, int c2, int c3) {
+  asm volatile(
+      "cp.async.bulk.tensor.4d.shared::cluster.global.mbarrier::complete_tx::bytes.multicast::cluster"
+      " [%0], [%1, {%4, %5, %6, %7}], [%2], %3;"
+      ::"r"(dst), "l"(reinterpret_cast<uint64_t>(m)), "r"(bar), "h"(cta_mask), "r"(c0), "r"(c1), "r"(c2), "r"(c3)
       : "memory");
 }
 __device__ __forceinline__ void tma_store_4d(const CUtensorMap* m, uint32_t src, int c0, int c1, int c2, int c3) {
@@ -235,6 +266,12 @@
 __device__ __forceinline__ void umma_commit(uint32_t bar) {
   asm volatile("tcgen05.commit.cta_group::1.mbarrier::arrive::one.shared::cluster.b64 [%0];" ::"r"(bar) : "memory");
 }
+__device__ __forceinline__ void umma_commit_multicast(uint32_t bar, uint16_t cta_mask) {
+  asm volatile("tcgen05.commit.cta_group::1.mbarrier::arrive::one.shared::cluster.multicast::cluster.b64 [%0], %1;" ::"r"(
+                   bar),
+               "h"(cta_mask)
+               : "memory");
+}
 
 template <int N>
 __device__ __forceinline__ void setmaxnreg_inc() { asm volatile("setmaxnreg.inc.sync.aligned.u32 %0;" ::"n"(N)); }
```

New measurement: 822.7, median of 6. About the same (+0.0%).
